# Michaelszeng/GCS-ADMM

Measured on NVIDIA B200. Metric: admm_iterations_per_second, higher is better.
Workload: dtype f64

## Files before the change

gcs-admm_b200/csrc/emulate.cpp:

```cpp
#define GCS_EMULATE 1
#include <stdio.h>
#include <stdlib.h>
#include <string.h>
#include "vertex_update.cuh"
#include "vertex_perf.cuh"

extern "C" int gcsemu_vertex_update_all(int nV, int nE, const int *poly_off, const double *polyA, const double *polyb,
                                        const int *he_off, const int *he_edge, const unsigned char *he_flags,
                                        const unsigned char *vtype, const double *cent, double *xc, const double *mu,
                                        const double *z, double *x_v, double *z_v, double *y_v, double rho, double mu_scale,
                                        double tol, int max_iter, int dcap, int mcap, long *total_iters, double *ws, double theta) {
    GcsGraphView G = {nV, nE, poly_off, polyA, polyb, he_off, he_edge, he_flags, vtype, cent};
    GcsStateView St = {xc, mu, z, x_v, z_v, y_v, ws, theta, 0.0};
    GcsScratchLayout L = gcs_scratch_layout(dcap, mcap);
    double *S = (double *)malloc(sizeof(double) * L.total);
    int fails = 0;
    long iters = 0;
    for (int v = 0; v < nV; ++v) {
        int status = 0;
        memset(S, getenv("GCSEMU_POISON") ? 0xFF : 0, sizeof(double) * L.total);
        iters += gcs_vertex_update(G, St, v, rho, mu_scale, tol, max_iter, L, S, 0, &status);
        if (status > 0 && status != 5) { fails++; if (getenv("GCSEMU_VERBOSE")) fprintf(stderr, "emu: vertex %d status %d\n", v, status); }
    }
    free(S);
    *total_iters = iters;
    return fails;
}
extern "C" int gcsemu_scratch_doubles(int dcap, int mcap) { return gcs_scratch_layout(dcap, mcap).total; }
extern "C" int gcsemu_ws_stride(int dcap, int mcap) { return gcs_ws_stride(gcs_scratch_layout(dcap, mcap)); }

template <bool INNER>
static int perf_all(int nV, int nE, const int *poly_off, const double *polyA, const double *polyb,
                    const int *he_off, const int *he_edge, const unsigned char *he_flags,
                    const unsigned char *vtype, const double *cent, double *xc, const double *mu,
                    const double *z, double *x_v, double *z_v, double *y_v, double rho, double mu_scale,
                    const int *vclass, const double *cls_tab, const int *cone_off, const double *cone,
                    const int *blk_off, const int *blk_he, const int *blk_edge, const int *blk_info, const int *tile_voff, int ntiles,
                    int cap_blocks, int cap_verts, int cap_cone, double *tstate, double *tn,
                    int inner_iters, double alpha, double kappa, double theta, const double *edge_delta, double *rin_tile) {
    GcsGraphView G = {nV, nE, poly_off, polyA, polyb, he_off, he_edge, he_flags, vtype, cent};
    GcsStateView St = {xc, mu, z, x_v, z_v, y_v, 0, 0.0, 0.0};
    GcsPerfLayout L = gcs_perf_layout(cap_blocks, cap_verts, cap_cone);
    const int nB = blk_off[nV];
    int *brec = (int *)calloc(4 * (size_t)(nB ? nB : 1), sizeof(int)), *vrec = (int *)calloc(GCS_VI_N * (size_t)nV, sizeof(int)), *trec = (int *)calloc(8 * (size_t)ntiles, sizeof(int));
    for (int b = 0; b < nB; ++b) { brec[4 * b] = blk_he[b]; brec[4 * b + 1] = blk_info[b]; brec[4 * b + 2] = blk_edge[b]; }
    for (int t = 0; t < ntiles; ++t) {
        const int a = tile_voff[t], b = tile_voff[t + 1];
        int *r = trec + 8 * t;
        r[0] = a; r[1] = b - a; r[2] = blk_off[a]; r[3] = blk_off[b] - blk_off[a]; r[4] = cone_off[a]; r[5] = cone_off[b] - cone_off[a];
        r[6] = he_off[a]; r[7] = he_off[b] - he_off[a];
        for (int hh = he_off[a]; hh < he_off[b]; ++hh) if (he_flags[hh] & GCS_HE_ZERO) r[7] |= 1 << 30;
        for (int v = a; v < b; ++v) {
            int *w = vrec + GCS_VI_N * v;
            w[GCS_VI_CONE] = cone_off[v] - cone_off[a]; w[GCS_VI_NV] = cone_off[v + 1] - cone_off[v]; w[GCS_VI_CLS] = vclass[v];
            w[GCS_VI_TERM] = vtype[v] != GCS_VT_GENERIC; w[GCS_VI_BLK] = blk_off[v] - blk_off[a]; w[GCS_VI_NB] = blk_off[v + 1] - blk_off[v];
            w[GCS_VI_ACTIVE] = 0; w[GCS_VI_HE] = he_off[v] - he_off[a];
        }
    }
    GcsPerfTables T = {vclass, cls_tab, cone_off, cone, blk_off, brec, vrec, trec, ntiles, tstate, tn, inner_iters, alpha, kappa, theta, edge_delta};
    Ctrl ctrl;
    memset(&ctrl, 0, sizeof ctrl);
    ctrl.rho = rho; ctrl.mu_scale = mu_scale;
    const int poison = getenv("GCSEMU_POISON") ? 0xFF : 0;
#pragma omp parallel
    {
        double *S = (double *)malloc(sizeof(double) * L.total);
#pragma omp for schedule(dynamic, 16)
        for (int t = 0; t < ntiles; ++t) {
            memset(S, poison, sizeof(double) * L.total);
            Ctrl local = ctrl;
            double rin = 0.0;
            gcs_perf_tile<INNER>(G, St, T, L, S, S + L.work, t, &local, 0, rin);
            if (rin_tile) rin_tile[t] = rin;
        }
        free(S);
    }
    free(brec); free(vrec); free(trec);
    for (int v = 0; v < nV; ++v)
        if (vtype[v] == GCS_VT_DEAD) { for (int k = 0; k < 4; ++k) { z_v[4 * v + k] = 0.0; x_v[4 * v + k] = cent[2 * v + (k & 1)]; } y_v[v] = 0.0; }
    return ntiles;
}

extern "C" int gcsemu_vertex_update_perf_all(int nV, int nE, const int *poly_off, const double *polyA, const double *polyb,
                                             const int *he_off, const int *he_edge, const unsigned char *he_flags,
                                             const unsigned char *vtype, const double *cent, double *xc, const double *mu,
                                             const double *z, double *x_v, double *z_v, double *y_v, double rho, double mu_scale,
                                             const int *vclass, const double *cls_tab, const int *cone_off, const double *cone,
                                             const int *blk_off, const int *blk_he, const int *blk_edge, const int *blk_info, const int *tile_voff, int ntiles,
                                             int cap_blocks, int cap_verts, int cap_cone, double *tstate, double *tn,
                                             int inner_iters, double alpha, double kappa, double theta, const double *edge_delta) {
    return perf_all<false>(nV, nE, poly_off, polyA, polyb, he_off, he_edge, he_flags, vtype, cent, xc, mu, z, x_v, z_v, y_v, rho, mu_scale,
                           vclass, cls_tab, cone_off, cone, blk_off, blk_he, blk_edge, blk_info, tile_voff, ntiles, cap_blocks, cap_verts,
                           cap_cone, tstate, tn, inner_iters, alpha, kappa, theta, edge_delta, nullptr);
}

extern "C" int gcsemu_vertex_update_perf_inner(int nV, int nE, const int *poly_off, const double *polyA, const double *polyb,
                                               const int *he_off, const int *he_edge, const unsigned char *he_flags,
                                               const unsigned char *vtype, const double *cent, double *xc, const double *mu,
                                               const double *z, double *x_v, double *z_v, double *y_v, double rho, double mu_scale,
                                               const int *vclass, const double *cls_tab, const int *cone_off, const double *cone,
                                               const int *blk_off, const int *blk_he, const int *blk_edge, const int *blk_info, const int *tile_voff, int ntiles,
                                               int cap_blocks, int cap_verts, int cap_cone, double *tstate, double *tn,
                                               int inner_iters, double alpha, double kappa, double theta, const double *edge_delta, double *inner_sq) {
    double *rin = (double *)calloc((size_t)(ntiles > 0 ? ntiles : 1), sizeof(double));
    const int r = perf_all<true>(nV, nE, poly_off, polyA, polyb, he_off, he_edge, he_flags, vtype, cent, xc, mu, z, x_v, z_v, y_v, rho, mu_scale,
                                 vclass, cls_tab, cone_off, cone, blk_off, blk_he, blk_edge, blk_info, tile_voff, ntiles, cap_blocks, cap_verts,
                                 cap_cone, tstate, tn, inner_iters, alpha, kappa, theta, edge_delta, rin);
    double s = 0.0;
    for (int t = 0; t < ntiles; ++t) s += rin[t];
    *inner_sq = s;
    free(rin);
    return r;
}

extern "C" void gcsemu_cone_project(const double *cone, int nv, const double *pts, int n, double *out) {
    for (int i = 0; i < n; ++i) gcs_cone_project(cone, nv, pts[3 * i], pts[3 * i + 1], pts[3 * i + 2], out[3 * i], out[3 * i + 1], out[3 * i + 2]);
}
```

gcs-admm_b200/csrc/gcsadmm.cu:

```cuda
#include <cuda_runtime.h>
#include <math.h>
#include <stdio.h>
#include <stdlib.h>
#include <string.h>
#include <new>
#include <nvtx3/nvToolsExt.h>

struct NvtxRange {
    explicit NvtxRange(const char *name) { nvtxRangePushA(name); }
    ~NvtxRange() { nvtxRangePop(); }
};

#include "../../include/gcsadmm.h"
#include "gcs_ctrl.h"
#include "vertex_update.cuh"
#include "vertex_perf.cuh"

#define GCS_VERSION "gcsadmm 0.1.0 (sm_100a)"
#define K1_MAX_WARPS 12
#define EDGE_THREADS 256

static thread_local char g_err[512] = "";
static int set_err(int code, const char *fmt, const char *a = "", const char *b = "") {
    snprintf(g_err, sizeof g_err, fmt, a, b);
    return code;
}
#define CK(call)                                                                                   \
    do {                                                                                           \
        cudaError_t e_ = (call);                                                                   \
        if (e_ != cudaSuccess) return set_err(GCS_E_CUDA, "%s: %s", #call, cudaGetErrorString(e_)); \
    } while (0)

#define GCS_MAX_PEERS 8
#define GCS_PEER_TIMEOUT_NS 20000000000ull
struct PeerComm {
    int halo_flag[GCS_MAX_PEERS];
    int sums_flag[GCS_MAX_PEERS];
    double sums_in[2][GCS_MAX_PEERS][NSUMS];
    int k;
    int error;
};
struct PeerView {
    int rank, world;
    unsigned neighbours;
    double *xc[GCS_MAX_PEERS];
    PeerComm *comm[GCS_MAX_PEERS];
    int nHown[GCS_MAX_PEERS], nHghost[GCS_MAX_PEERS];
};

struct PeerPush { const int *send_he, *send_rank, *send_slot; int nsend; const PeerView *PV; unsigned int *ticket; };

struct GcsHandle {
    int device;
    cudaStream_t stream, own_stream;
    GcsParams p;
    int nV, nE, nHown, nHghost;
    int nP;
    long long n_x, n_mu;
    int dcap, mcap;
    GcsScratchLayout L;
    int k1_smem, k1_blocks, k1_warps, edge_blocks, edge_per_edge, edge_minb, edge_coop, coop_blocks;
    int *poly_off, *he_off, *he_edge, *edge_he_tail, *edge_he_head;
    double *polyA, *polyb, *cent;
    unsigned char *he_flags, *vtype, *edge_counted;
    int *vprob, *prob_eoff; long long *prob_nx, *prob_nmu;
    int *he_prob_host;
    unsigned int *ticket;
    unsigned int *push_ticket;
    double *xc, *mu, *z, *x_v, *z_v, *y_v;
    double *ws;
    double *partials;
    double *hist;
    int hist_cap;
    Ctrl *ctrl;
    Ctrl *ctrl_host;
    cudaEvent_t ev[4];
    void *flush_buf; size_t flush_bytes;
    int perf_on, perf_smem, perf_threads, perf_grid;
    int inner_on;
    GcsPerfLayout PL;
    GcsPerfTables PT;
    long long perf_nblocks;
    int *p_vclass, *p_cone_off, *p_blk_off, *p_blk_rec, *p_vrec, *p_tile_rec; double *p_cls_tab, *p_cone, *p_tstate, *p_tn, *p_edge_delta, *p_edge_cent, *p_tile_res;
    cudaGraphExec_t graph_exec; int graph_iters;
    int peer_on, rank, world, nsend;
    PeerView PV; PeerView *PV_dev;
    PeerComm *comm;
    void *ipc_opened[2 * GCS_MAX_PEERS];
    int *send_he, *send_rank, *send_slot;
};

__global__ void __launch_bounds__(K1_MAX_WARPS * 32)
vertex_kernel(GcsGraphView G, GcsStateView St, Ctrl *ctrl_all, const int *__restrict__ vprob, GcsScratchLayout L, double tol, int max_iter) {
    extern __shared__ double smem[];
    const int lane = threadIdx.x & 31, warp = threadIdx.x >> 5;
    const int v = blockIdx.x * (blockDim.x >> 5) + warp;
    if (v >= G.nV) return;
    Ctrl *ctrl = ctrl_all + (vprob ? vprob[v] : 0);
    if (ctrl->stop && !ctrl->ignore_stop) return;
    double *S = smem + (size_t)warp * L.total;
    int status = 0;
    const int iters = gcs_vertex_update(G, St, v, ctrl->rho, ctrl->mu_scale, tol, max_iter, L, S, lane, &status);
    if (lane == 0) {
        if (iters) atomicAdd(&ctrl->inner_iters, (unsigned long long)iters);
        if (status > 0 && status != 5) atomicAdd(&ctrl->inner_fail, 1);
        if (status < 0) atomicAdd(&ctrl->skipped, 1ull);
    }
}

__device__ __forceinline__ unsigned long long gcs_globaltimer() { unsigned long long t; asm volatile("mov.u64 %0, %globaltimer;" : "=l"(t)); return t; }

__device__ __forceinline__ void peer_push(const double *xc, const int *__restrict__ send_he, const int *__restrict__ send_rank,
                                          const int *__restrict__ send_slot, int nsend, const PeerView &PV) {
    const int k = PV.comm[PV.rank]->k + 1, par = k & 1;
    for (int i = threadIdx.x; i < 5 * nsend; i += blockDim.x) {
        const int j = i / 5, c = i - 5 * j, q = send_rank[j];
        PV.xc[q][5 * ((size_t)PV.nHown[q] + (size_t)par * PV.nHghost[q] + send_slot[j]) + c] = __ldcg(xc + 5 * (size_t)send_he[j] + c);
    }
    __threadfence_system();
    __syncthreads();
    if (threadIdx.x < PV.world && ((PV.neighbours >> threadIdx.x) & 1u)) *(volatile int *)&PV.comm[threadIdx.x]->halo_flag[PV.rank] = k;
}
__device__ __forceinline__ void peer_wait_halo(const PeerView &PV) {
    PeerComm *me = PV.comm[PV.rank];
    const int k = me->k + 1, p = threadIdx.x;
    if (p < PV.world && ((PV.neighbours >> p) & 1u)) {
        const unsigned long long t0 = gcs_globaltimer();
        while (*(volatile int *)&me->halo_flag[p] < k)
            if (gcs_globaltimer() - t0 > GCS_PEER_TIMEOUT_NS) { me->error = 1; break; }
        __threadfence_system();
    }
    __syncthreads();
}

template <bool INNER>
__global__ void __launch_bounds__(GCS_PERF_THREADS, 4)
vertex_perf_kernel(GcsGraphView G, GcsStateView St, GcsPerfTables T, Ctrl *ctrl_all, const int *__restrict__ vprob, GcsPerfLayout L, PeerPush P) {
    extern __shared__ __align__(16) double smem[];
    __shared__ __align__(8) unsigned long long bar[2];
    if (!vprob && ctrl_all->stop && !ctrl_all->ignore_stop) return;
    int tile = blockIdx.x;
    if (tile >= T.ntiles) return;
    double *const stage0 = smem + L.work;
#define STAGE(b) (stage0 + (b) * L.stage)
    if (threadIdx.x == 0) {
        gcs_mbar_init(&bar[0], 1);
        gcs_mbar_init(&bar[1], 1);
        gcs_perf_stage(T, L, STAGE(0), tile, &bar[0]);
    }
    __syncthreads();
    unsigned phase = 0;
    double rin = 0.0;
    for (int buf = 0; tile < T.ntiles; tile += gridDim.x, buf ^= 1) {
        const int next = tile + gridDim.x;
        if (threadIdx.x == 0 && next < T.ntiles) {
            gcs_bulk_wait_read();
            gcs_perf_stage(T, L, STAGE(buf ^ 1), next, &bar[buf ^ 1]);
        }
        gcs_mbar_wait(&bar[buf], (phase >> buf) & 1u);
        phase ^= 1u << buf;
        gcs_perf_tile<INNER>(G, St, T, L, smem, STAGE(buf), tile, ctrl_all, vprob, rin);
    }
    if (threadIdx.x == 0) gcs_bulk_wait_read();
#undef STAGE
    if (INNER) {
#pragma unroll
        for (int o = 16; o; o >>= 1) rin += __shfl_xor_sync(0xffffffffu, rin, o);
        __syncthreads();
        if ((threadIdx.x & 31) == 0) smem[L.rin + (threadIdx.x >> 5)] = rin;
        __syncthreads();
        if (threadIdx.x == 0) {
            double s = 0.0;
            for (int w2 = 0; w2 < (int)(blockDim.x >> 5); ++w2) s += smem[L.rin + w2];
            T.tile_res[blockIdx.x] = s;
        }
    }
    if (P.PV) {
        __shared__ int is_last;
        __threadfence();
        __syncthreads();
        if (threadIdx.x == 0) is_last = (atomicAdd(P.ticket, 1u) == gridDim.x - 1);
        __syncthreads();
        if (is_last) {
            __threadfence();
            peer_push(St.xc, P.send_he, P.send_rank, P.send_slot, P.nsend, *P.PV);
            if (threadIdx.x == 0) *P.ticket = 0u;
        }
    }
}
__global__ void perf_init_dead_kernel(GcsGraphView G, GcsStateView St) {
    const int v = blockIdx.x * blockDim.x + threadIdx.x;
    if (v >= G.nV || G.vtype[v] != GCS_VT_DEAD) return;
    for (int k = 0; k < 4; ++k) { St.z_v[4 * (size_t)v + k] = 0.0; St.x_v[4 * (size_t)v + k] = G.cent[2 * (size_t)v + (k & 1)]; }
    St.y_v[v] = 0.0;
}

__device__ void control_apply(Ctrl *ctrl, const GcsParams &p, long long n_x, long long n_mu, double *hist, int hist_cap) {
    const int it = ctrl->it + 1;
    const double *s = ctrl->sums;
    const double rho = ctrl->rho;
    const double pri = sqrt(s[0]);
    const double dual = rho * sqrt(2.0 * s[1]);
    double rho_new = rho, scale = 1.0;
    const bool may = it < p.frac * p.max_it && (p.adapt_every <= 1 || it % p.adapt_every == 0);
    if (pri >= p.nu * dual && may) { rho_new = rho * p.tau_incr; scale = 1.0 / p.tau_incr; }
    else if (dual >= p.nu * pri && may) { rho_new = rho * (1.0 / p.tau_decr); scale = p.tau_incr; }
    const double nAx = sqrt(s[2]), nBz = sqrt(2.0 * s[3]), nmu = scale * sqrt(s[4]);
    const double eps_pri = sqrt((double)n_x) * p.eps_abs + p.eps_rel * fmax(nAx, nBz);
    const double eps_dual = sqrt((double)n_mu) * p.eps_abs + p.eps_rel * nmu;
    const double inner = s[6] < 0.0 ? -1.0 : sqrt(s[6]);
    const double pri_g = s[7] < 0.0 ? -1.0 : sqrt(s[7]), dual_g = s[8] < 0.0 ? -1.0 : rho * sqrt(2.0 * s[8]);
    ctrl->pri_g = pri_g; ctrl->dual_g = dual_g;
    ctrl->it = it; ctrl->pri = pri; ctrl->dual = dual; ctrl->eps_pri = eps_pri; ctrl->eps_dual = eps_dual; ctrl->inner = inner;
    ctrl->rho = rho_new; ctrl->mu_scale = scale;
    if (it < hist_cap) { hist[it] = rho_new; hist[hist_cap + it] = pri; hist[2 * hist_cap + it] = dual; }
    if (s[5] != 0.0 || !isfinite(pri) || !isfinite(dual)) { ctrl->diverged = 1; ctrl->stop = 1; return; }
    const bool ref = p.stop_ref && pri_g >= 0.0 && dual_g >= 0.0;
    const bool opt = p.abs_stop ? (inner >= 0.0 && fmax(fmax(ref ? pri_g : pri, ref ? dual_g : dual), inner) < p.abs_tol)
                                : (pri < eps_pri && dual < eps_dual);
    if (opt) { ctrl->opt = 1; ctrl->stop = 1; }
}

__device__ __forceinline__ void edge_finish(double r2, double dz2, double x2, double z2, double m2, double r2g, double dz2g, Ctrl *ctrl, double *__restrict__ partials,
                                            unsigned int *ticket, int fuse, const GcsParams &p, long long n_x, long long n_mu, double *hist,
                                            int hist_cap, const PeerView *PVp, const double *__restrict__ tile_res, int ntiles) {
    double bad = 0;
    if (!isfinite(r2) || !isfinite(dz2) || !isfinite(x2) || !isfinite(z2)) bad = 1.0;
    __shared__ double sh[EDGE_THREADS][9];
    __shared__ int is_last;
    double vals[8] = {r2, dz2, x2, z2, m2, bad, r2g, dz2g};
#pragma unroll
    for (int q = 0; q < 8; ++q)
#pragma unroll
        for (int o = 16; o; o >>= 1) vals[q] += __shfl_xor_sync(0xffffffffu, vals[q], o);
    const int lane = threadIdx.x & 31, warp = threadIdx.x >> 5;
    if (lane == 0)
#pragma unroll
        for (int q = 0; q < 8; ++q) sh[warp][q] = vals[q];
    __syncthreads();
    if (threadIdx.x < 8) {
        double s = 0.0;
        for (int w2 = 0; w2 < EDGE_THREADS / 32; ++w2) s += sh[w2][threadIdx.x];
        partials[(size_t)blockIdx.x * NSUMS + (threadIdx.x < 6 ? threadIdx.x : threadIdx.x + 1)] = s;
        __threadfence();
    }
    __syncthreads();
    if (threadIdx.x == 0) {
        const unsigned int t = atomicAdd(ticket, 1u);
        is_last = (t == gridDim.x - 1);
    }
    __syncthreads();
    if (!is_last) return;
    __threadfence();
    double acc[9] = {0, 0, 0, 0, 0, 0, 0, 0, 0};
    for (int b = threadIdx.x; b < (int)gridDim.x; b += blockDim.x)
#pragma unroll
        for (int q = 0; q < 9; ++q) if (q != 6) acc[q] += __ldcg(partials + (size_t)b * NSUMS + q);
    if (tile_res) { for (int b = threadIdx.x; b < ntiles; b += blockDim.x) acc[6] += __ldcg(tile_res + b); }
    else if (ntiles < 0 && threadIdx.x == 0) acc[6] = -1.0;
#pragma unroll
    for (int q = 0; q < 9; ++q) sh[threadIdx.x][q] = acc[q];
    __syncthreads();
    for (int st = EDGE_THREADS / 2; st > 0; st >>= 1) {
        if (threadIdx.x < st)
#pragma unroll
            for (int q = 0; q < 9; ++q) sh[threadIdx.x][q] += sh[threadIdx.x + st][q];
        __syncthreads();
    }
    if (threadIdx.x < 9) ctrl->sums[threadIdx.x] = sh[0][threadIdx.x];
    __syncthreads();
    if (fuse == 2) {
        const int me = PVp->rank, world = PVp->world, k = PVp->comm[me]->k + 1, par = k & 1;
        if (threadIdx.x < 9)
            for (int q = 0; q < world; ++q) PVp->comm[q]->sums_in[par][me][threadIdx.x] = sh[0][threadIdx.x];
        __threadfence_system();
        __syncthreads();
        if (threadIdx.x < world) { *(volatile int *)&PVp->comm[threadIdx.x]->sums_flag[me] = k; }
        if (threadIdx.x == 0) *ticket = 0u;
        return;
    }
    if (threadIdx.x == 0) {
        *ticket = 0u;
        if (fuse) control_apply(ctrl, p, n_x, n_mu, hist, hist_cap);
    }
}

__global__ void __launch_bounds__(EDGE_THREADS, 6)
edge_kernel(int nE, int nHown, const int *__restrict__ edge_he_tail, const int *__restrict__ edge_he_head,
            const unsigned char *__restrict__ edge_counted, const double *__restrict__ xc, double *__restrict__ mu,
            double *__restrict__ z, Ctrl *ctrl, double *__restrict__ partials, unsigned int *ticket, int fuse,
            GcsParams p, long long n_x, long long n_mu, double *hist, int hist_cap, int nHghost, const PeerView *PVp, const double *__restrict__ tile_res, int ntiles) {
    if (ctrl->stop && !ctrl->ignore_stop) return;
    if (fuse == 2) peer_wait_halo(*PVp);
    const double ms = ctrl->mu_scale, oa = p.outer_alpha, ob = 1.0 - p.outer_alpha;
    const int gpar = fuse == 2 ? ((PVp->comm[PVp->rank]->k + 1) & 1) * nHghost : 0;
    double r2 = 0, dz2 = 0, x2 = 0, z2 = 0, m2 = 0;
    const unsigned n = 5u * (unsigned)nE, stride = gridDim.x * blockDim.x;
    for (unsigned i = blockIdx.x * blockDim.x + threadIdx.x; i < n; i += stride) {
        const unsigned e = i / 5u, c = i - 5u * e;
        const int ht = edge_he_tail[e], hh = edge_he_head[e];
        const bool ot = ht < nHown, oh = hh < nHown;
        const unsigned it_ = 5u * (unsigned)(ot ? ht : ht + gpar) + c, ih_ = 5u * (unsigned)(oh ? hh : hh + gpar) + c;
        const double xt = xc[it_], xh = xc[ih_], zo = z[i];
        const double mt = ot ? mu[it_] : 0.0, mh = oh ? mu[ih_] : 0.0;
        const double w = edge_counted ? (double)edge_counted[e] : 1.0;
        double at = xt, ah = xh;
        if (oa != 1.0) { at = oa * xt + ob * zo; ah = oa * xh + ob * zo; }
        const double zn = 0.5 * (at + ah), dd = zn - zo;
        z[i] = zn;
        dz2 += w * dd * dd; z2 += w * zn * zn;
        if (ot) { const double r = zn - xt, mn = ms * mt + (zn - at); mu[it_] = mn; r2 += r * r; x2 += xt * xt; m2 += mn * mn; }
        if (oh) { const double r = zn - xh, mn = ms * mh + (zn - ah); mu[ih_] = mn; r2 += r * r; x2 += xh * xh; m2 += mn * mn; }
    }
    const double none = (blockIdx.x == 0 && threadIdx.x == 0) ? -1.0 : 0.0;
    edge_finish(r2, dz2, x2, z2, m2, none, none, ctrl, partials, ticket, fuse, p, n_x, n_mu, hist, hist_cap, PVp, tile_res, ntiles);
}

template <int MINB, bool OA, bool GRES>
__global__ void __launch_bounds__(EDGE_THREADS, MINB)
edge_frames_kernel(int nE, int nHown, const int *__restrict__ edge_he_tail, const int *__restrict__ edge_he_head,
                   const unsigned char *__restrict__ edge_counted, const double *__restrict__ edge_delta, const double *__restrict__ edge_cent, const double *__restrict__ xc,
                   double *__restrict__ mu, double *__restrict__ z, Ctrl *ctrl, double *__restrict__ partials, unsigned int *ticket, int fuse,
                   GcsParams p, long long n_x, long long n_mu, double *hist, int hist_cap, int nHghost, const PeerView *PVp, const double *__restrict__ tile_res, int ntiles) {
    if (ctrl->stop && !ctrl->ignore_stop) return;
    if (fuse == 2) peer_wait_halo(*PVp);
    const double ms = ctrl->mu_scale, oa = p.outer_alpha, ob = 1.0 - p.outer_alpha;
    const int gpar = fuse == 2 ? ((PVp->comm[PVp->rank]->k + 1) & 1) * nHghost : 0;
    double r2 = 0, dz2 = 0, x2 = 0, z2 = 0, m2 = 0, r2g = 0, dz2g = 0;
    if (!GRES && blockIdx.x == 0 && threadIdx.x == 0) r2g = dz2g = -1.0;
    const int estride = gridDim.x * blockDim.x;
    int e = blockIdx.x * blockDim.x + threadIdx.x, ht = 0, hh = 0;
    if (e < nE) { ht = edge_he_tail[e]; hh = edge_he_head[e]; }
    for (; e < nE; e += estride) {
        const int en = e + estride, ht_ = ht, hh_ = hh;
        if (en < nE) { ht = edge_he_tail[en]; hh = edge_he_head[en]; }
        const bool ot = ht_ < nHown, oh = hh_ < nHown;
        const double *pt = xc + 5 * (size_t)(ot ? ht_ : ht_ + gpar), *ph = xc + 5 * (size_t)(oh ? hh_ : hh_ + gpar);
        double xt[5], xh[5], zo[5], mt[5], mh[5];
#pragma unroll
        for (int c = 0; c < 5; ++c) { xt[c] = pt[c]; xh[c] = ph[c]; zo[c] = z[5 * (size_t)e + c]; }
        if (MINB == 2) {
#pragma unroll
            for (int c = 0; c < 5; ++c) { mt[c] = ot ? mu[5 * (size_t)ht_ + c] : 0.0; mh[c] = oh ? mu[5 * (size_t)hh_ + c] : 0.0; }
        }
        const double d0 = edge_delta ? edge_delta[2 * (size_t)e] : 0.0, d1 = edge_delta ? edge_delta[2 * (size_t)e + 1] : 0.0;
        const double w = edge_counted ? (double)edge_counted[e] : 1.0;
        double zn[5], bz[5], at[5], ah[5];
#pragma unroll
        for (int c = 0; c < 5; ++c) { at[c] = xt[c]; ah[c] = xh[c]; }
        if (OA) {
            const double bo[5] = {zo[0], zo[1], zo[2] - d0 * zo[4], zo[3] - d1 * zo[4], zo[4]};
#pragma unroll
            for (int c = 0; c < 5; ++c) { at[c] = oa * xt[c] + ob * bo[c]; ah[c] = oa * xh[c] + ob * zo[c]; }
        }
        zn[0] = 0.5 * (ah[0] + at[0]); zn[1] = 0.5 * (ah[1] + at[1]);
        const double q0 = ah[2] + at[2], q1 = ah[3] + at[3], q2 = ah[4] + at[4] - (d0 * at[2] + d1 * at[3]);
        zn[4] = (q2 + 0.5 * (d0 * q0 + d1 * q1)) / (2.0 + 0.5 * (d0 * d0 + d1 * d1));
        zn[2] = 0.5 * (q0 + d0 * zn[4]); zn[3] = 0.5 * (q1 + d1 * zn[4]);
        bz[0] = zn[0]; bz[1] = zn[1]; bz[2] = zn[2] - d0 * zn[4]; bz[3] = zn[3] - d1 * zn[4]; bz[4] = zn[4];
        double dd[5];
#pragma unroll
        for (int c = 0; c < 5; ++c) { dd[c] = zn[c] - zo[c]; z[5 * (size_t)e + c] = zn[c]; }
        const double db2 = dd[2] - d0 * dd[4], db3 = dd[3] - d1 * dd[4];
        dz2 += 0.5 * w * (2.0 * (dd[0] * dd[0] + dd[1] * dd[1] + dd[4] * dd[4]) + dd[2] * dd[2] + dd[3] * dd[3] + db2 * db2 + db3 * db3);
        z2 += 0.5 * w * (2.0 * (zn[0] * zn[0] + zn[1] * zn[1] + zn[4] * zn[4]) + zn[2] * zn[2] + zn[3] * zn[3] + bz[2] * bz[2] + bz[3] * bz[3]);
        double cu0 = 0.0, cu1 = 0.0, cw0 = 0.0, cw1 = 0.0;
        if (GRES) {
            cu0 = edge_cent[2 * (size_t)e]; cu1 = edge_cent[2 * (size_t)e + 1]; cw0 = cu0 - d0; cw1 = cu1 - d1;
            const double g0 = dd[0] + dd[4] * cu0, g1 = dd[1] + dd[4] * cu1, g2 = dd[2] + dd[4] * cw0, g3 = dd[3] + dd[4] * cw1;
            dz2g += w * (g0 * g0 + g1 * g1 + g2 * g2 + g3 * g3 + dd[4] * dd[4]);
        }
        if (MINB > 2) asm volatile("" ::: "memory");
        if (ot) {
            if (MINB > 2) {
#pragma unroll
                for (int c = 0; c < 5; ++c) mt[c] = mu[5 * (size_t)ht_ + c];
            }
#pragma unroll
            for (int c = 0; c < 5; ++c) { const double r = bz[c] - xt[c], mn = ms * mt[c] + (bz[c] - at[c]); mu[5 * (size_t)ht_ + c] = mn; r2 += r * r; x2 += xt[c] * xt[c]; m2 += mn * mn; }
            if (GRES) {
                const double ry = bz[4] - xt[4], a0 = bz[0] - xt[0] + ry * cu0, a1 = bz[1] - xt[1] + ry * cu1, a2 = bz[2] - xt[2] + ry * cu0, a3 = bz[3] - xt[3] + ry * cu1;
                r2g += a0 * a0 + a1 * a1 + a2 * a2 + a3 * a3 + ry * ry;
            }
        }
        if (oh) {
            if (MINB > 2) {
#pragma unroll
                for (int c = 0; c < 5; ++c) mh[c] = mu[5 * (size_t)hh_ + c];
            }
#pragma unroll
            for (int c = 0; c < 5; ++c) { const double r = zn[c] - xh[c], mn = ms * mh[c] + (zn[c] - ah[c]); mu[5 * (size_t)hh_ + c] = mn; r2 += r * r; x2 += xh[c] * xh[c]; m2 += mn * mn; }
            if (GRES) {
                const double ry = zn[4] - xh[4], a0 = zn[0] - xh[0] + ry * cu0, a1 = zn[1] - xh[1] + ry * cu1, a2 = zn[2] - xh[2] + ry * cw0, a3 = zn[3] - xh[3] + ry * cw1;
                r2g += a0 * a0 + a1 * a1 + a2 * a2 + a3 * a3 + ry * ry;
            }
        }
    }
    edge_finish(r2, dz2, x2, z2, m2, r2g, dz2g, ctrl, partials, ticket, fuse, p, n_x, n_mu, hist, hist_cap, PVp, tile_res, ntiles);
}

#define COOP_WARPS (EDGE_THREADS / 32)
#define COOP_SMEM_DOUBLES (COOP_WARPS * 5 * 160)
template <bool OA, int MINB>
__global__ void __launch_bounds__(EDGE_THREADS, MINB)
edge_coop_kernel(int nE, const int *__restrict__ edge_he_tail, const int *__restrict__ edge_he_head, const double *__restrict__ edge_delta,
                 const double *__restrict__ xc, double *__restrict__ mu, double *__restrict__ z, Ctrl *ctrl, double *__restrict__ partials,
                 unsigned int *ticket, int fuse, GcsParams p, long long n_x, long long n_mu, double *hist, int hist_cap,
                 const double *__restrict__ tile_res, int ntiles) {
    extern __shared__ __align__(16) double coop_sm[];
    if (ctrl->stop && !ctrl->ignore_stop) return;
    const double ms = ctrl->mu_scale, oa = p.outer_alpha, ob = 1.0 - p.outer_alpha;
    const int lane = threadIdx.x & 31, warp = threadIdx.x >> 5;
    double *xtS = coop_sm + (size_t)warp * 800, *xhS = xtS + 160, *zoS = xtS + 320, *mtS = xtS + 480, *mhS = xtS + 640;
    double r2 = 0, dz2 = 0, x2 = 0, z2 = 0, m2 = 0, r2g = 0, dz2g = 0;
    if (blockIdx.x == 0 && threadIdx.x == 0) r2g = dz2g = -1.0;
    const int nchunks = (nE + 31) >> 5;
    for (int chunk = blockIdx.x * COOP_WARPS + warp; chunk < nchunks; chunk += gridDim.x * COOP_WARPS) {
        const int e = (chunk << 5) + lane;
        const bool valid = e < nE;
        const int ht = valid ? edge_he_tail[e] : 0, hh = valid ? edge_he_head[e] : 0;
        const double d0 = valid && edge_delta ? edge_delta[2 * (size_t)e] : 0.0, d1 = valid && edge_delta ? edge_delta[2 * (size_t)e + 1] : 0.0;
        const size_t zbase = (size_t)chunk * 160;
        double vx[5], vh[5], vz[5], vm[5], vn[5];
        int tj[5], hj[5];
#pragma unroll
        for (int k = 0; k < 5; ++k) {
            const int i = lane + 32 * k, j = i / 5, c = i - 5 * j;
            tj[k] = 5 * __shfl_sync(0xffffffffu, ht, j) + c;
            hj[k] = 5 * __shfl_sync(0xffffffffu, hh, j) + c;
        }
#pragma unroll
        for (int k = 0; k < 5; ++k) {
            const int i = lane + 32 * k;
            vx[k] = xc[tj[k]]; vh[k] = xc[hj[k]]; vm[k] = mu[tj[k]]; vn[k] = mu[hj[k]];
            vz[k] = zbase + i < 5 * (size_t)nE ? z[zbase + i] : 0.0;
        }
#pragma unroll
        for (int k = 0; k < 5; ++k) {
            const int i = lane + 32 * k;
            xtS[i] = vx[k]; xhS[i] = vh[k]; mtS[i] = vm[k]; mhS[i] = vn[k]; zoS[i] = vz[k];
        }
        __syncwarp();
        double xt[5], xh[5], zo[5], mt[5], mh[5];
#pragma unroll
        for (int c = 0; c < 5; ++c) { xt[c] = xtS[5 * lane + c]; xh[c] = xhS[5 * lane + c]; zo[c] = zoS[5 * lane + c]; mt[c] = mtS[5 * lane + c]; mh[c] = mhS[5 * lane + c]; }
        __syncwarp();
        double zn[5], bz[5], at[5], ah[5];
#pragma unroll
        for (int c = 0; c < 5; ++c) { at[c] = xt[c]; ah[c] = xh[c]; }
        if (OA) {
            const double bo[5] = {zo[0], zo[1], zo[2] - d0 * zo[4], zo[3] - d1 * zo[4], zo[4]};
#pragma unroll
            for (int c = 0; c < 5; ++c) { at[c] = oa * xt[c] + ob * bo[c]; ah[c] = oa * xh[c] + ob * zo[c]; }
        }
        zn[0] = 0.5 * (ah[0] + at[0]); zn[1] = 0.5 * (ah[1] + at[1]);
        const double q0 = ah[2] + at[2], q1 = ah[3] + at[3], q2 = ah[4] + at[4] - (d0 * at[2] + d1 * at[3]);
        zn[4] = (q2 + 0.5 * (d0 * q0 + d1 * q1)) / (2.0 + 0.5 * (d0 * d0 + d1 * d1));
        zn[2] = 0.5 * (q0 + d0 * zn[4]); zn[3] = 0.5 * (q1 + d1 * zn[4]);
        bz[0] = zn[0]; bz[1] = zn[1]; bz[2] = zn[2] - d0 * zn[4]; bz[3] = zn[3] - d1 * zn[4]; bz[4] = zn[4];
        double dd[5];
#pragma unroll
        for (int c = 0; c < 5; ++c) { dd[c] = zn[c] - zo[c]; zoS[5 * lane + c] = zn[c]; }
        const double db2 = dd[2] - d0 * dd[4], db3 = dd[3] - d1 * dd[4];
        if (valid) {
            dz2 += 0.5 * (2.0 * (dd[0] * dd[0] + dd[1] * dd[1] + dd[4] * dd[4]) + dd[2] * dd[2] + dd[3] * dd[3] + db2 * db2 + db3 * db3);
            z2 += 0.5 * (2.0 * (zn[0] * zn[0] + zn[1] * zn[1] + zn[4] * zn[4]) + zn[2] * zn[2] + zn[3] * zn[3] + bz[2] * bz[2] + bz[3] * bz[3]);
        }
#pragma unroll
        for (int c = 0; c < 5; ++c) {
            const double r = bz[c] - xt[c], mn = ms * mt[c] + (bz[c] - at[c]);
            mtS[5 * lane + c] = mn;
            if (valid) { r2 += r * r; x2 += xt[c] * xt[c]; m2 += mn * mn; }
        }
#pragma unroll
        for (int c = 0; c < 5; ++c) {
            const double r = zn[c] - xh[c], mn = ms * mh[c] + (zn[c] - ah[c]);
            mhS[5 * lane + c] = mn;
            if (valid) { r2 += r * r; x2 += xh[c] * xh[c]; m2 += mn * mn; }
        }
        __syncwarp();
#pragma unroll
        for (int k = 0; k < 5; ++k) {
            const int i = lane + 32 * k, j = i / 5;
            if ((chunk << 5) + j < nE) { z[zbase + i] = zoS[i]; mu[tj[k]] = mtS[i]; mu[hj[k]] = mhS[i]; }
        }
        __syncwarp();
    }
    edge_finish(r2, dz2, x2, z2, m2, r2g, dz2g, ctrl, partials, ticket, fuse, p, n_x, n_mu, hist, hist_cap, nullptr, tile_res, ntiles);
}

__global__ void __launch_bounds__(1024)
peer_push_kernel(const double *__restrict__ xc, const int *__restrict__ send_he, const int *__restrict__ send_rank,
                 const int *__restrict__ send_slot, int nsend, Ctrl *ctrl, const PeerView *PVp) {
    if (ctrl->stop && !ctrl->ignore_stop) return;
    peer_push(xc, send_he, send_rank, send_slot, nsend, *PVp);
}
__global__ void peer_control_kernel(Ctrl *ctrl, GcsParams p, long long n_x, long long n_mu, double *hist, int hist_cap, const PeerView *PVp) {
    if (ctrl->stop && !ctrl->ignore_stop) return;
    const PeerView &PV = *PVp;
    PeerComm *me = PV.comm[PV.rank];
    const int k = me->k + 1, par = k & 1, q = threadIdx.x;
    if (q < PV.world) {
        const unsigned long long t0 = gcs_globaltimer();
        while (*(volatile int *)&me->sums_flag[q] < k)
            if (gcs_globaltimer() - t0 > GCS_PEER_TIMEOUT_NS) { me->error = 1; break; }
    }
    __threadfence_system();
    __syncwarp();
    if (threadIdx.x == 0) {
        for (int j = 0; j < 9; ++j) {
            double s = 0.0;
            for (int r = 0; r < PV.world; ++r) s += *(volatile double *)&me->sums_in[par][r][j];
            ctrl->sums[j] = s;
        }
        if (me->error) { ctrl->diverged = 1; ctrl->stop = 1; }
        else control_apply(ctrl, p, n_x, n_mu, hist, hist_cap);
        me->k = k;
    }
}

__global__ void control_kernel(Ctrl *ctrl, GcsParams p, long long n_x, long long n_mu, double *hist, int hist_cap) {
    if (threadIdx.x != 0 || blockIdx.x != 0) return;
    if (ctrl->stop && !ctrl->ignore_stop) return;
    control_apply(ctrl, p, n_x, n_mu, hist, hist_cap);
}

#define BATCH_THREADS 128
__global__ void __launch_bounds__(BATCH_THREADS)
batched_edge_kernel(int nP, const int *__restrict__ prob_eoff, int nHown, const int *__restrict__ edge_he_tail,
                    const int *__restrict__ edge_he_head, const double *__restrict__ xc, double *__restrict__ mu,
                    double *__restrict__ z, Ctrl *ctrl_all, GcsParams p, const long long *__restrict__ prob_nx,
                    const long long *__restrict__ prob_nmu, double *hist, int hist_cap) {
    __shared__ double sh[BATCH_THREADS / 32][6];
    for (int q = blockIdx.x; q < nP; q += gridDim.x) {
        Ctrl *ctrl = ctrl_all + q;
        if (ctrl->stop && !ctrl->ignore_stop) continue;
        const double ms = ctrl->mu_scale;
        double r2 = 0, dz2 = 0, x2 = 0, z2 = 0, m2 = 0, bad = 0;
        for (int e = prob_eoff[q] + threadIdx.x; e < prob_eoff[q + 1]; e += blockDim.x) {
            const int ht = edge_he_tail[e], hh = edge_he_head[e];
            double xt[5], xh[5], zn[5];
#pragma unroll
            for (int c = 0; c < 5; ++c) { xt[c] = xc[5 * (size_t)ht + c]; xh[c] = xc[5 * (size_t)hh + c]; }
#pragma unroll
            for (int c = 0; c < 5; ++c) {
                const double zo = z[5 * (size_t)e + c];
                zn[c] = 0.5 * (xt[c] + xh[c]);
                const double dd = zn[c] - zo;
                dz2 += dd * dd; z2 += zn[c] * zn[c];
                z[5 * (size_t)e + c] = zn[c];
            }
#pragma unroll
            for (int c = 0; c < 5; ++c) {
                const double rt = zn[c] - xt[c], mt = ms * mu[5 * (size_t)ht + c] + rt;
                mu[5 * (size_t)ht + c] = mt; r2 += rt * rt; x2 += xt[c] * xt[c]; m2 += mt * mt;
                const double rh = zn[c] - xh[c], mh = ms * mu[5 * (size_t)hh + c] + rh;
                mu[5 * (size_t)hh + c] = mh; r2 += rh * rh; x2 += xh[c] * xh[c]; m2 += mh * mh;
            }
        }
        if (!isfinite(r2) || !isfinite(dz2) || !isfinite(x2) || !isfinite(z2)) bad = 1.0;
        double vals[6] = {r2, dz2, x2, z2, m2, bad};
#pragma unroll
        for (int k = 0; k < 6; ++k)
#pragma unroll
            for (int o = 16; o; o >>= 1) vals[k] += __shfl_xor_sync(0xffffffffu, vals[k], o);
        const int lane = threadIdx.x & 31, warp = threadIdx.x >> 5;
        if (lane == 0)
            for (int k = 0; k < 6; ++k) sh[warp][k] = vals[k];
        __syncthreads();
        if (threadIdx.x == 0) {
            for (int k = 0; k < 6; ++k) {
                double sum = 0.0;
                for (int w2 = 0; w2 < BATCH_THREADS / 32; ++w2) sum += sh[w2][k];
                ctrl->sums[k] = sum;
            }
            control_apply(ctrl, p, prob_nx[q], prob_nmu[q], hist + (size_t)q * 3 * hist_cap, hist_cap);
        }
        __syncthreads();
    }
}
__global__ void set_ignore_kernel(Ctrl *ctrl, int nP, int v) {
    for (int q = blockIdx.x * blockDim.x + threadIdx.x; q < nP; q += gridDim.x * blockDim.x) ctrl[q].ignore_stop = v;
}

extern "C" const char *gcsadmm_version(void) { return GCS_VERSION; }
extern "C" const char *gcsadmm_last_error(void) { return g_err; }
extern "C" int gcsadmm_device_count(void) {
    int n = 0;
    if (cudaGetDeviceCount(&n) != cudaSuccess) { cudaGetLastError(); return 0; }
    return n;
}
extern "C" void gcsadmm_default_params(GcsParams *p) {
    p->rho0 = 1.0; p->tau_incr = 2.0; p->tau_decr = 2.0; p->nu = 10.0; p->frac = 0.1;
    p->eps_abs = 1e-4; p->eps_rel = 1e-3; p->max_it = 1000; p->inner_tol = 1e-8; p->inner_max_iter = 60;
    p->check_every = 8; p->abs_stop = 0; p->abs_tol = 1e-4; p->warm_theta = 1e-3; p->zero_tol = 1e-12;
    p->outer_alpha = 1.0; p->use_graph = 1; p->adapt_every = 1; p->stop_ref = 0;
}
extern "C" int gcsadmm_scratch_bytes(int max_live_degree, int max_rows) {
    return (int)(gcs_scratch_layout(max_live_degree, max_rows).total * sizeof(double));
}

template <typename T>
static int upload(T **dst, const T *src, size_t n) {
    if (n == 0) n = 1, src = nullptr;
    cudaError_t e = cudaMalloc((void **)dst, n * sizeof(T));
    if (e != cudaSuccess) { char nb[32]; snprintf(nb, sizeof nb, "%zu", n * sizeof(T)); return set_err(GCS_E_NOMEM, "cudaMalloc(%s bytes): %s", nb, cudaGetErrorString(e)); }
    if (src) { e = cudaMemcpy(*dst, src, n * sizeof(T), cudaMemcpyHostToDevice); if (e != cudaSuccess) return set_err(GCS_E_CUDA, "cudaMemcpy H2D: %s", cudaGetErrorString(e)); }
    else cudaMemset(*dst, 0, n * sizeof(T));
    return 0;
}

static int reset_ctrl(GcsHandle *h) {
    Ctrl c; memset(&c, 0, sizeof c);
    c.rho = h->p.rho0; c.mu_scale = 1.0;
    double first[3] = {h->p.rho0, 0.0, 0.0};
    for (int q = 0; q < h->nP; ++q) {
        h->ctrl_host[q] = c;
        for (int k = 0; k < 3; ++k)
            CK(cudaMemcpyAsync(h->hist + ((size_t)q * 3 + k) * h->hist_cap, &first[k], sizeof(double), cudaMemcpyHostToDevice, h->stream));
    }
    CK(cudaMemcpyAsync(h->ctrl, h->ctrl_host, sizeof(Ctrl) * h->nP, cudaMemcpyHostToDevice, h->stream));
    CK(cudaStreamSynchronize(h->stream));
    return 0;
}

static void free_perf(GcsHandle *h) {
    void *pp[] = {h->p_vclass, h->p_cone_off, h->p_blk_off, h->p_blk_rec, h->p_vrec, h->p_tile_rec, h->p_cls_tab, h->p_cone, h->p_tstate, h->p_tn, h->p_edge_delta, h->p_edge_cent, h->p_tile_res};
    for (void *q : pp) if (q) cudaFree(q);
    h->p_vclass = h->p_cone_off = h->p_blk_off = h->p_blk_rec = h->p_vrec = h->p_tile_rec = nullptr;
    h->p_cls_tab = h->p_cone = h->p_tstate = h->p_tn = h->p_edge_delta = h->p_edge_cent = h->p_tile_res = nullptr;
    h->perf_on = 0;
}
static void drop_graph(GcsHandle *h) {
    if (h->graph_exec) { cudaGraphExecDestroy(h->graph_exec); h->graph_exec = nullptr; }
    h->graph_iters = 0;
}

extern "C" int gcsadmm_destroy(GcsHandle *h) {
    if (!h) return 0;
    cudaSetDevice(h->device);
    void *ptrs[] = {h->poly_off, h->he_off, h->he_edge, h->edge_he_tail, h->edge_he_head, h->polyA, h->polyb, h->cent,
                    h->he_flags, h->vtype, h->edge_counted, h->xc, h->mu, h->z, h->x_v, h->z_v, h->y_v, h->ws, h->partials, h->hist, h->ctrl,
                    h->vprob, h->prob_eoff, h->prob_nx, h->prob_nmu};
    for (void *p : ptrs) if (p) cudaFree(p);
    if (h->ctrl_host) cudaFreeHost(h->ctrl_host);
    free(h->he_prob_host);
    if (h->flush_buf) cudaFree(h->flush_buf);
    if (h->graph_exec) cudaGraphExecDestroy(h->graph_exec);
    for (void *m : h->ipc_opened) if (m) cudaIpcCloseMemHandle(m);
    { void *pp[] = {h->comm, h->send_he, h->send_rank, h->send_slot, h->PV_dev}; for (void *q : pp) if (q) cudaFree(q); }
    if (h->ticket) cudaFree(h->ticket);
    if (h->push_ticket) cudaFree(h->push_ticket);
    free_perf(h);
    for (int i = 0; i < 4; ++i) if (h->ev[i]) cudaEventDestroy(h->ev[i]);
    if (h->own_stream) cudaStreamDestroy(h->own_stream);
    delete h;
    return 0;
}

static int validate_graph(const GcsGraph *g) {
    if (!g->poly_off || !g->polyA || !g->polyb || !g->he_off || !g->vtype || !g->cent) return set_err(GCS_E_INVALID, "null graph array%s", "");
    if (g->nH_own < 0 || g->nH_ghost < 0 || g->he_off[0] != 0 || g->he_off[g->nV] != g->nH_own) return set_err(GCS_E_INVALID, "he_off does not span nH_own%s", "");
    if (g->nH_own && (!g->he_edge || !g->he_flags)) return set_err(GCS_E_INVALID, "null half-edge array%s", "");
    if (g->nE && (!g->edge_he_tail || !g->edge_he_head)) return set_err(GCS_E_INVALID, "null edge array%s", "");
    if (g->poly_off[0] != 0) return set_err(GCS_E_INVALID, "poly_off[0] != 0%s", "");
    for (int v = 0; v < g->nV; ++v) {
        if (g->he_off[v + 1] < g->he_off[v] || g->poly_off[v + 1] < g->poly_off[v]) return set_err(GCS_E_INVALID, "offsets not monotone%s", "");
        if (g->vtype[v] > 3) return set_err(GCS_E_INVALID, "bad vertex type%s", "");
    }
    for (int hh = 0; hh < g->nH_own; ++hh) if (g->he_edge[hh] < 0 || g->he_edge[hh] >= g->nE) return set_err(GCS_E_INVALID, "he_edge out of range%s", "");
    const int nHall = g->nH_own + g->nH_ghost;
    for (int e = 0; e < g->nE; ++e)
        if (g->edge_he_tail[e] < 0 || g->edge_he_tail[e] >= nHall || g->edge_he_head[e] < 0 || g->edge_he_head[e] >= nHall)
            return set_err(GCS_E_INVALID, "edge_he_tail / edge_he_head out of range%s", "");
    return 0;
}

static int create_impl(GcsHandle *h, const GcsGraph *g) {
    int dcap = 1, mcap = 1;
    for (int v = 0; v < g->nV; ++v) {
        int d = 0;
        for (int hh = g->he_off[v]; hh < g->he_off[v + 1]; ++hh) if (!(g->he_flags[hh] & GCS_HE_FLAG_ZERO)) d++;
        if (d > dcap) dcap = d;
        int m = g->poly_off[v + 1] - g->poly_off[v];
        if (m > mcap) mcap = m;
        if (g->vtype[v] == GCS_VT_GENERIC && d < 2) return set_err(GCS_E_INVALID, "inconsistent presolve flags (generic vertex with < 2 live half-edges)%s", "");
    }
    h->dcap = dcap; h->mcap = mcap;
    h->L = gcs_scratch_layout(dcap, mcap);
    cudaDeviceProp prop;
    CK(cudaGetDeviceProperties(&prop, h->device));
    {
        const size_t per_warp = (size_t)h->L.total * sizeof(double);
        const size_t budget = prop.sharedMemPerBlockOptin;
        int w = (int)(budget / per_warp);
        if (w < 1) return set_err(GCS_E_INVALID, "vertex program too large for shared memory (max live degree / polytope rows too high)%s", "");
        if (w > K1_MAX_WARPS) w = K1_MAX_WARPS;
        h->k1_warps = w;
        h->k1_smem = (int)(w * per_warp);
    }
    CK(cudaFuncSetAttribute(vertex_kernel, cudaFuncAttributeMaxDynamicSharedMemorySize, h->k1_smem));
    CK(cudaFuncSetAttribute(vertex_kernel, cudaFuncAttributePreferredSharedMemoryCarveout, 100));
    h->k1_blocks = (g->nV + h->k1_warps - 1) / h->k1_warps;
    {
        const long long need = (5ll * g->nE + EDGE_THREADS - 1) / EDGE_THREADS;
        const char *bps = getenv("GCS_EDGE_BLOCKS_PER_SM"), *ek = getenv("GCS_EDGE_KERNEL");
        h->edge_per_edge = !(ek && !strcmp(ek, "per_scalar"));
        h->edge_coop = !(ek && (!strcmp(ek, "per_edge") || !strcmp(ek, "per_scalar")));
        h->coop_blocks = prop.multiProcessorCount * (bps && atoi(bps) > 0 ? atoi(bps) : 2);
        const char *mb = getenv("GCS_EDGE_MINB");
        h->edge_minb = mb && atoi(mb) >= 2 && atoi(mb) <= 4 ? atoi(mb) : 2;
        if (h->edge_coop) {
            const int smb = (int)(sizeof(double) * COOP_SMEM_DOUBLES);
            CK(cudaFuncSetAttribute(edge_coop_kernel<false, 2>, cudaFuncAttributeMaxDynamicSharedMemorySize, smb));
            CK(cudaFuncSetAttribute(edge_coop_kernel<true, 2>, cudaFuncAttributeMaxDynamicSharedMemorySize, smb));
            CK(cudaFuncSetAttribute(edge_coop_kernel<false, 3>, cudaFuncAttributeMaxDynamicSharedMemorySize, smb));
            CK(cudaFuncSetAttribute(edge_coop_kernel<true, 3>, cudaFuncAttributeMaxDynamicSharedMemorySize, smb));
        }
        const long long cap = (long long)prop.multiProcessorCount * (bps && atoi(bps) > 0 ? atoi(bps) : (h->edge_per_edge ? 4 : 6));
        h->edge_blocks = (int)(need < 1 ? 1 : (need > cap ? cap : need));
    }
    CK(cudaStreamCreateWithFlags(&h->own_stream, cudaStreamNonBlocking));
    h->stream = h->own_stream;
    const size_t M = (size_t)g->poly_off[g->nV], Hall = (size_t)g->nH_own + g->nH_ghost;
    int rc = 0;
#define UP(field, src, n) if (!rc) rc = upload(&h->field, src, (size_t)(n))
    UP(poly_off, g->poly_off, g->nV + 1); UP(polyA, g->polyA, 2 * M); UP(polyb, g->polyb, M);
    UP(he_off, g->he_off, g->nV + 1); UP(he_edge, g->he_edge, g->nH_own); UP(he_flags, g->he_flags, g->nH_own);
    UP(edge_he_tail, g->edge_he_tail, g->nE); UP(edge_he_head, g->edge_he_head, g->nE);
    UP(vtype, g->vtype, g->nV); UP(cent, g->cent, 2 * (size_t)g->nV);
    if (g->edge_counted) UP(edge_counted, g->edge_counted, g->nE);
    UP(xc, (const double *)nullptr, 5 * (Hall + (size_t)g->nH_ghost));
    UP(mu, (const double *)nullptr, 5 * (size_t)g->nH_own); UP(z, (const double *)nullptr, 5 * (size_t)g->nE);
    UP(x_v, (const double *)nullptr, 4 * (size_t)g->nV); UP(z_v, (const double *)nullptr, 4 * (size_t)g->nV); UP(y_v, (const double *)nullptr, g->nV);
    if (h->p.warm_theta > 0.0) UP(ws, (const double *)nullptr, (size_t)g->nV * gcs_ws_stride(h->L));
    UP(partials, (const double *)nullptr, (size_t)h->edge_blocks * NSUMS);
    UP(ticket, (const unsigned int *)nullptr, 1);
    UP(push_ticket, (const unsigned int *)nullptr, 1);
    h->hist_cap = h->p.max_it + 2;
    UP(hist, (const double *)nullptr, 3 * (size_t)h->hist_cap * h->nP);
#undef UP
    if (rc) return rc;
    CK(cudaMalloc((void **)&h->ctrl, sizeof(Ctrl) * h->nP));
    CK(cudaMallocHost((void **)&h->ctrl_host, sizeof(Ctrl) * h->nP));
    if (h->nP > 1) {
        int *vp = (int *)malloc(sizeof(int) * g->nV);
        long long *nx = (long long *)malloc(sizeof(long long) * h->nP), *nm = (long long *)malloc(sizeof(long long) * h->nP);
        h->he_prob_host = (int *)malloc(sizeof(int) * (size_t)(g->nH_own > 0 ? g->nH_own : 1));
        if (!vp || !nx || !nm || !h->he_prob_host) { free(vp); free(nx); free(nm); return set_err(GCS_E_NOMEM, "out of host memory%s", ""); }
        for (int q = 0; q < h->nP; ++q) {
            for (int v = g->prob_voff[q]; v < g->prob_voff[q + 1]; ++v) {
                vp[v] = q;
                for (int hh = g->he_off[v]; hh < g->he_off[v + 1]; ++hh) h->he_prob_host[hh] = q;
            }
            const long long nv = g->prob_voff[q + 1] - g->prob_voff[q], ne = g->prob_eoff[q + 1] - g->prob_eoff[q];
            nx[q] = 9 * nv + 18 * ne; nm[q] = 10 * ne;
        }
        rc = upload(&h->vprob, vp, (size_t)g->nV);
        if (!rc) rc = upload(&h->prob_eoff, g->prob_eoff, (size_t)h->nP + 1);
        if (!rc) rc = upload(&h->prob_nx, nx, (size_t)h->nP);
        if (!rc) rc = upload(&h->prob_nmu, nm, (size_t)h->nP);
        free(vp); free(nx); free(nm);
        if (rc) return rc;
    }
    for (int i = 0; i < 4; ++i) CK(cudaEventCreate(&h->ev[i]));
    return reset_ctrl(h);
}

extern "C" int gcsadmm_create(const GcsGraph *g, const GcsParams *p, int device, GcsHandle **out) {
    NvtxRange nvtx_("gcsadmm_create");
    if (!g || !out) return set_err(GCS_E_INVALID, "null argument%s", "");
    *out = nullptr;
    if (g->n != 2) return set_err(GCS_E_INVALID, "the CUDA path is specialised to n = 2 (2-D GCS)%s", "");
    if (g->nV <= 0 || g->nE < 0) return set_err(GCS_E_INVALID, "empty graph%s", "");
    int rc = validate_graph(g);
    if (rc) return rc;
    int ndev = 0;
    if (cudaGetDeviceCount(&ndev) != cudaSuccess || ndev == 0) { cudaGetLastError(); return set_err(GCS_E_CUDA, "no CUDA device: libgcsadmm has no CPU path%s", ""); }
    if (device < 0 || device >= ndev) return set_err(GCS_E_INVALID, "bad device index%s", "");
    const int nP = g->nP > 1 ? g->nP : 1;
    if (nP > 1 && (g->nH_ghost > 0 || !g->prob_voff || !g->prob_eoff)) return set_err(GCS_E_INVALID, "batched problems need prob_voff / prob_eoff and cannot be vertex-partitioned%s", "");
    CK(cudaSetDevice(device));
    GcsHandle *h = new (std::nothrow) GcsHandle();
    if (!h) return set_err(GCS_E_NOMEM, "out of host memory%s", "");
    memset(h, 0, sizeof *h);
    h->device = device;
    if (p) h->p = *p; else gcsadmm_default_params(&h->p);
    if (h->p.check_every < 1) h->p.check_every = 1;
    if (!(h->p.outer_alpha > 0.0 && h->p.outer_alpha < 2.0)) h->p.outer_alpha = 1.0;
    h->nV = g->nV; h->nE = g->nE; h->nHown = g->nH_own; h->nHghost = g->nH_ghost;
    h->nP = nP;
    h->n_x = g->n_x_global ? g->n_x_global : 9LL * g->nV + 18LL * g->nE;
    h->n_mu = g->n_mu_global ? g->n_mu_global : 10LL * g->nE;
    rc = create_impl(h, g);
    if (rc) { gcsadmm_destroy(h); return rc; }
    *out = h;
    return 0;
}

extern "C" int gcsadmm_set_stream(GcsHandle *h, void *s, int external) {
    if (!h) return set_err(GCS_E_INVALID, "null handle%s", "");
    CK(cudaSetDevice(h->device));
    CK(cudaStreamSynchronize(h->stream));
    h->stream = external ? (cudaStream_t)s : h->own_stream;
    drop_graph(h);
    return 0;
}

static GcsGraphView graph_view(const GcsHandle *h) {
    GcsGraphView G; G.nV = h->nV; G.nE = h->nE; G.poly_off = h->poly_off; G.polyA = h->polyA; G.polyb = h->polyb;
    G.he_off = h->he_off; G.he_edge = h->he_edge; G.he_flags = h->he_flags; G.vtype = h->vtype; G.cent = h->cent;
    return G;
}
static GcsStateView state_view(const GcsHandle *h) {
    GcsStateView S; S.xc = h->xc; S.mu = h->mu; S.z = h->z; S.x_v = h->x_v; S.z_v = h->z_v; S.y_v = h->y_v;
    S.ws = h->ws; S.theta = h->p.warm_theta; S.zero_tol = h->p.zero_tol;
    return S;
}
static int launch_k1(GcsHandle *h) {
    if (h->perf_on) {
        PeerPush P = {h->send_he, h->send_rank, h->send_slot, h->nsend, h->peer_on ? h->PV_dev : nullptr, h->push_ticket};
        if (h->inner_on) vertex_perf_kernel<true><<<h->perf_grid, h->perf_threads, h->perf_smem, h->stream>>>(graph_view(h), state_view(h), h->PT, h->ctrl, h->vprob, h->PL, P);
        else vertex_perf_kernel<false><<<h->perf_grid, h->perf_threads, h->perf_smem, h->stream>>>(graph_view(h), state_view(h), h->PT, h->ctrl, h->vprob, h->PL, P);
        return 0;
    }
    vertex_kernel<<<h->k1_blocks, h->k1_warps * 32, h->k1_smem, h->stream>>>(graph_view(h), state_view(h), h->ctrl, h->vprob, h->L, h->p.inner_tol, h->p.inner_max_iter);
    return 0;
}
#define INNER_ARGS(h) ((h)->perf_on && (h)->inner_on ? (h)->p_tile_res : nullptr), ((h)->perf_on && (h)->nP == 1 ? ((h)->inner_on ? (h)->perf_grid : -1) : 0)
static int launch_edge(GcsHandle *h, int fuse) {
    if (h->nP > 1) {
        const int blocks = h->nP < 148 * 16 ? h->nP : 148 * 16;
        batched_edge_kernel<<<blocks, BATCH_THREADS, 0, h->stream>>>(h->nP, h->prob_eoff, h->nHown, h->edge_he_tail, h->edge_he_head, h->xc, h->mu, h->z,
                                                                     h->ctrl, h->p, h->prob_nx, h->prob_nmu, h->hist, h->hist_cap);
        return 0;
    }
    if (h->edge_coop && h->nHghost == 0 && !h->edge_counted && !(h->perf_on && h->inner_on)) {
        const int nchunks = (h->nE + 31) / 32;
        int blocks = (nchunks + COOP_WARPS - 1) / COOP_WARPS;
        if (blocks > h->coop_blocks) blocks = h->coop_blocks;
        if (blocks < 1) blocks = 1;
        const size_t sm = sizeof(double) * COOP_SMEM_DOUBLES;
#define EDGE_COOP(OA, MINB) edge_coop_kernel<OA, MINB><<<blocks, EDGE_THREADS, sm, h->stream>>>(h->nE, h->edge_he_tail, h->edge_he_head, h->perf_on ? h->p_edge_delta : nullptr, \
            h->xc, h->mu, h->z, h->ctrl, h->partials, h->ticket, fuse, h->p, h->n_x, h->n_mu, h->hist, h->hist_cap, INNER_ARGS(h))
        if (h->p.outer_alpha != 1.0) { if (h->edge_minb >= 3) EDGE_COOP(true, 3); else EDGE_COOP(true, 2); }
        else { if (h->edge_minb >= 3) EDGE_COOP(false, 3); else EDGE_COOP(false, 2); }
#undef EDGE_COOP
        return 0;
    }
    if ((h->perf_on && h->p_edge_delta) || h->edge_per_edge) {
        int blocks = (h->nE + EDGE_THREADS - 1) / EDGE_THREADS;
        if (blocks > h->edge_blocks) blocks = h->edge_blocks;
        if (blocks < 1) blocks = 1;
        const bool gres = h->perf_on && h->inner_on && h->p_edge_delta && h->p_edge_cent;
#define EDGE_FRAMES(MINB) if (gres) { if (h->p.outer_alpha != 1.0) EDGE_FRAMES_(MINB, true, true); else EDGE_FRAMES_(MINB, false, true); } \
                          else { if (h->p.outer_alpha != 1.0) EDGE_FRAMES_(MINB, true, false); else EDGE_FRAMES_(MINB, false, false); }
#define EDGE_FRAMES_(MINB, OA, GRES) edge_frames_kernel<MINB, OA, GRES><<<blocks, EDGE_THREADS, 0, h->stream>>>(h->nE, h->nHown, h->edge_he_tail, h->edge_he_head, h->edge_counted, \
            h->perf_on ? h->p_edge_delta : nullptr, h->perf_on ? h->p_edge_cent : nullptr, h->xc, h->mu, h->z, h->ctrl, h->partials, h->ticket, fuse, h->p, h->n_x, h->n_mu, h->hist, h->hist_cap, h->nHghost, h->PV_dev, INNER_ARGS(h))
        if (h->edge_minb == 4) { EDGE_FRAMES(4); } else if (h->edge_minb == 3) { EDGE_FRAMES(3); } else { EDGE_FRAMES(2); }
#undef EDGE_FRAMES
#undef EDGE_FRAMES_
        return 0;
    }
    edge_kernel<<<h->edge_blocks, EDGE_THREADS, 0, h->stream>>>(h->nE, h->nHown, h->edge_he_tail, h->edge_he_head, h->edge_counted, h->xc, h->mu, h->z, h->ctrl,
                                                                h->partials, h->ticket, fuse, h->p, h->n_x, h->n_mu, h->hist, h->hist_cap, h->nHghost, h->PV_dev, INNER_ARGS(h));
    return 0;
}
static int launch_ctrl(GcsHandle *h) {
    if (h->nP > 1) return 0;
    control_kernel<<<1, 32, 0, h->stream>>>(h->ctrl, h->p, h->n_x, h->n_mu, h->hist, h->hist_cap);
    return 0;
}
static void launch_rest(GcsHandle *h) {
    if (!h->peer_on) { launch_edge(h, 1); return; }
    if (!h->perf_on) peer_push_kernel<<<1, 1024, 0, h->stream>>>(h->xc, h->send_he, h->send_rank, h->send_slot, h->nsend, h->ctrl, h->PV_dev);
    launch_edge(h, 2);
    peer_control_kernel<<<1, 32, 0, h->stream>>>(h->ctrl, h->p, h->n_x, h->n_mu, h->hist, h->hist_cap, h->PV_dev);
}
static void launch_iteration(GcsHandle *h) { launch_k1(h); launch_rest(h); }
static int launch_chunk(GcsHandle *h, int iters) {
    NvtxRange nvtx_("gcsadmm: chunk of ADMM iterations");
    if (!h->p.use_graph || h->stream != h->own_stream || iters < 2 || iters != h->p.check_every) { for (int i = 0; i < iters; ++i) launch_iteration(h); return 0; }
    if (!h->graph_exec || h->graph_iters != iters) {
        drop_graph(h);
        cudaGraph_t graph = nullptr;
        CK(cudaStreamBeginCapture(h->stream, cudaStreamCaptureModeThreadLocal));
        for (int i = 0; i < iters; ++i) launch_iteration(h);
        CK(cudaStreamEndCapture(h->stream, &graph));
        cudaError_t e = cudaGraphInstantiate(&h->graph_exec, graph, 0);
        cudaGraphDestroy(graph);
        if (e != cudaSuccess) { h->graph_exec = nullptr; return set_err(GCS_E_CUDA, "cudaGraphInstantiate: %s", cudaGetErrorString(e)); }
        h->graph_iters = iters;
    }
    CK(cudaGraphLaunch(h->graph_exec, h->stream));
    return 0;
}
static int set_ignore_stop(GcsHandle *h, int v) {
    if (h->nP > 1) { set_ignore_kernel<<<(h->nP + 255) / 256, 256, 0, h->stream>>>(h->ctrl, h->nP, v); return 0; }
    CK(cudaMemcpyAsync((char *)h->ctrl + offsetof(Ctrl, ignore_stop), &v, sizeof(int), cudaMemcpyHostToDevice, h->stream));
    return 0;
}
static int fetch_ctrl(GcsHandle *h) {
    CK(cudaMemcpyAsync(h->ctrl_host, h->ctrl, sizeof(Ctrl) * h->nP, cudaMemcpyDeviceToHost, h->stream));
    CK(cudaStreamSynchronize(h->stream));
    CK(cudaGetLastError());
    return 0;
}
static void fill_status_one(const Ctrl *c, GcsStatus *st) {
    st->iterations = c->it; st->converged = c->opt; st->diverged = c->diverged; st->inner_fail = c->inner_fail;
    st->inner_iters = (int64_t)c->inner_iters; st->skipped = (int64_t)c->skipped; st->rho = c->rho; st->pri_res = c->pri; st->dual_res = c->dual;
    st->eps_pri = c->eps_pri; st->eps_dual = c->eps_dual; st->inner_res = c->inner; st->pri_res_ref = c->pri_g >= 0.0 ? c->pri_g : c->pri; st->dual_res_ref = c->dual_g >= 0.0 ? c->dual_g : c->dual;
}
static void fill_status(const GcsHandle *h, GcsStatus *st) {
    fill_status_one(h->ctrl_host, st);
    for (int q = 1; q < h->nP; ++q) {
        GcsStatus t; fill_status_one(h->ctrl_host + q, &t);
        if (t.iterations > st->iterations) st->iterations = t.iterations;
        st->converged = st->converged && t.converged; st->diverged = st->diverged || t.diverged;
        st->inner_fail += t.inner_fail; st->inner_iters += t.inner_iters; st->skipped += t.skipped;
        if (t.pri_res > st->pri_res) { st->pri_res = t.pri_res; st->eps_pri = t.eps_pri; }
        if (t.dual_res > st->dual_res) { st->dual_res = t.dual_res; st->eps_dual = t.eps_dual; }
        if (t.inner_res > st->inner_res) st->inner_res = t.inner_res;
        if (t.pri_res_ref > st->pri_res_ref) st->pri_res_ref = t.pri_res_ref;
        if (t.dual_res_ref > st->dual_res_ref) st->dual_res_ref = t.dual_res_ref;
    }
}
static bool all_stopped(const GcsHandle *h) {
    for (int q = 0; q < h->nP; ++q) if (!h->ctrl_host[q].stop) return false;
    return true;
}
static bool any_diverged(const GcsHandle *h) {
    for (int q = 0; q < h->nP; ++q) if (h->ctrl_host[q].diverged) return true;
    return false;
}

extern "C" int gcsadmm_vertex_update(GcsHandle *h) { if (!h) return set_err(GCS_E_INVALID, "null handle%s", ""); CK(cudaSetDevice(h->device)); launch_k1(h); CK(cudaGetLastError()); return 0; }
extern "C" int gcsadmm_edge_update(GcsHandle *h) { if (!h) return set_err(GCS_E_INVALID, "null handle%s", ""); CK(cudaSetDevice(h->device)); launch_edge(h, 0); CK(cudaGetLastError()); return 0; }
extern "C" int gcsadmm_control(GcsHandle *h) { if (!h) return set_err(GCS_E_INVALID, "null handle%s", ""); CK(cudaSetDevice(h->device)); launch_ctrl(h); CK(cudaGetLastError()); return 0; }
extern "C" int gcsadmm_sums_device_ptr(GcsHandle *h, void **p) { if (!h || !p) return set_err(GCS_E_INVALID, "null argument%s", ""); *p = (char *)h->ctrl + offsetof(Ctrl, sums); return 0; }
extern "C" int gcsadmm_xc_device_ptr(GcsHandle *h, void **p) { if (!h || !p) return set_err(GCS_E_INVALID, "null argument%s", ""); *p = h->xc; return 0; }

extern "C" int gcsadmm_step(GcsHandle *h, int k) {
    if (!h) return set_err(GCS_E_INVALID, "null handle%s", "");
    CK(cudaSetDevice(h->device));
    int rc = set_ignore_stop(h, 1); if (rc) return rc;
    while (k > 0) {
        const int chunk = k < h->p.check_every ? k : h->p.check_every;
        rc = launch_chunk(h, chunk); if (rc) return rc;
        k -= chunk;
    }
    rc = set_ignore_stop(h, 0); if (rc) return rc;
    CK(cudaGetLastError());
    return fetch_ctrl(h);
}

extern "C" int gcsadmm_run(GcsHandle *h, int max_iters, GcsStatus *st) {
    NvtxRange nvtx_("gcsadmm_run");
    if (!h) return set_err(GCS_E_INVALID, "null handle%s", "");
    CK(cudaSetDevice(h->device));
    int rc = fetch_ctrl(h); if (rc) return rc;
    int done = 0;
    while (done < max_iters && !all_stopped(h)) {
        int chunk = h->p.check_every;
        if (chunk > max_iters - done) chunk = max_iters - done;
        rc = launch_chunk(h, chunk); if (rc) return rc;
        CK(cudaGetLastError());
        rc = fetch_ctrl(h); if (rc) return rc;
        done += chunk;
        if (h->perf_on && h->nP == 1 && h->p.abs_stop) {
            const int want = fmax(h->ctrl_host->pri, h->ctrl_host->dual) < 4.0 * h->p.abs_tol;
            if (want != h->inner_on) { h->inner_on = want; drop_graph(h); }
        }
    }
    if (st) fill_status(h, st);
    if (any_diverged(h)) return set_err(GCS_E_DIVERGED, "non-finite residuals (divergence)%s", "");
    return 0;
}

extern "C" int gcsadmm_get_status(GcsHandle *h, GcsStatus *st) {
    if (!h || !st) return set_err(GCS_E_INVALID, "null argument%s", "");
    CK(cudaSetDevice(h->device));
    int rc = fetch_ctrl(h); if (rc) return rc;
    fill_status(h, st);
    return 0;
}

extern "C" int gcsadmm_get_problem_status(GcsHandle *h, int problem, GcsStatus *st) {
    if (!h || !st || problem < 0 || problem >= h->nP) return set_err(GCS_E_INVALID, "bad argument%s", "");
    CK(cudaSetDevice(h->device));
    int rc = fetch_ctrl(h); if (rc) return rc;
    fill_status_one(h->ctrl_host + problem, st);
    return 0;
}
extern "C" int gcsadmm_get_problem_history(GcsHandle *h, int problem, double *rho, double *pri, double *dual, int cap) {
    if (!h || problem < 0 || problem >= h->nP) return set_err(GCS_E_INVALID, "bad argument%s", "");
    CK(cudaSetDevice(h->device));
    int rc = fetch_ctrl(h); if (rc) return rc;
    int n = h->ctrl_host[problem].it + 1;
    if (n > h->hist_cap) n = h->hist_cap;
    if (n > cap) n = cap;
    double *dst[3] = {rho, pri, dual};
    for (int k = 0; k < 3; ++k) if (dst[k]) CK(cudaMemcpy(dst[k], h->hist + ((size_t)problem * 3 + k) * h->hist_cap, sizeof(double) * n, cudaMemcpyDeviceToHost));
    return n;
}
extern "C" int gcsadmm_get_history(GcsHandle *h, double *rho, double *pri, double *dual, int cap) {
    if (!h) return set_err(GCS_E_INVALID, "null handle%s", "");
    CK(cudaSetDevice(h->device));
    int rc = fetch_ctrl(h); if (rc) return rc;
    int n = h->ctrl_host->it + 1;
    if (n > h->hist_cap) n = h->hist_cap;
    if (n > cap) n = cap;
    double *dst[3] = {rho, pri, dual};
    for (int q = 0; q < 3; ++q) if (dst[q]) CK(cudaMemcpy(dst[q], h->hist + (size_t)q * h->hist_cap, sizeof(double) * n, cudaMemcpyDeviceToHost));
    return n;
}

extern "C" int gcsadmm_get_solution(GcsHandle *h, double *x_v, double *z_v, double *y_v, double *z_e) {
    NvtxRange nvtx_("gcsadmm_get_solution");
    if (!h) return set_err(GCS_E_INVALID, "null handle%s", "");
    CK(cudaSetDevice(h->device));
    CK(cudaStreamSynchronize(h->stream));
    if (x_v) CK(cudaMemcpy(x_v, h->x_v, sizeof(double) * 4 * h->nV, cudaMemcpyDeviceToHost));
    if (z_v) CK(cudaMemcpy(z_v, h->z_v, sizeof(double) * 4 * h->nV, cudaMemcpyDeviceToHost));
    if (y_v) CK(cudaMemcpy(y_v, h->y_v, sizeof(double) * h->nV, cudaMemcpyDeviceToHost));
    if (z_e) CK(cudaMemcpy(z_e, h->z, sizeof(double) * 5 * h->nE, cudaMemcpyDeviceToHost));
    return 0;
}

extern "C" int gcsadmm_get_state(GcsHandle *h, double *xc, double *mu, double *z, double *rho, int *it) {
    if (!h) return set_err(GCS_E_INVALID, "null handle%s", "");
    CK(cudaSetDevice(h->device));
    int rc = fetch_ctrl(h); if (rc) return rc;
    if (xc) CK(cudaMemcpy(xc, h->xc, sizeof(double) * 5 * ((size_t)h->nHown + h->nHghost), cudaMemcpyDeviceToHost));
    if (mu) {
        CK(cudaMemcpy(mu, h->mu, sizeof(double) * 5 * (size_t)h->nHown, cudaMemcpyDeviceToHost));
        if (h->nP > 1) { for (size_t hh = 0; hh < (size_t)h->nHown; ++hh) { const double s = h->ctrl_host[h->he_prob_host[hh]].mu_scale; if (s != 1.0) for (int c = 0; c < 5; ++c) mu[5 * hh + c] *= s; } }
        else { const double s = h->ctrl_host->mu_scale; if (s != 1.0) for (size_t i = 0; i < 5 * (size_t)h->nHown; ++i) mu[i] *= s; }
    }
    if (z) CK(cudaMemcpy(z, h->z, sizeof(double) * 5 * (size_t)h->nE, cudaMemcpyDeviceToHost));
    if (rho) *rho = h->ctrl_host->rho;
    if (it) *it = h->ctrl_host->it;
    return 0;
}

extern "C" int gcsadmm_set_state(GcsHandle *h, const double *xc, const double *mu, const double *z, double rho, int it) {
    if (!h) return set_err(GCS_E_INVALID, "null handle%s", "");
    CK(cudaSetDevice(h->device));
    int rc = fetch_ctrl(h); if (rc) return rc;
    if (xc) CK(cudaMemcpy(h->xc, xc, sizeof(double) * 5 * ((size_t)h->nHown + h->nHghost), cudaMemcpyHostToDevice));
    if (mu) CK(cudaMemcpy(h->mu, mu, sizeof(double) * 5 * (size_t)h->nHown, cudaMemcpyHostToDevice));
    if (z) CK(cudaMemcpy(h->z, z, sizeof(double) * 5 * (size_t)h->nE, cudaMemcpyHostToDevice));
    for (int q = 0; q < h->nP; ++q) { Ctrl &c = h->ctrl_host[q]; c.rho = rho; c.it = it; c.mu_scale = 1.0; c.stop = 0; c.opt = 0; c.diverged = 0; }
    CK(cudaMemcpy(h->ctrl, h->ctrl_host, sizeof(Ctrl) * h->nP, cudaMemcpyHostToDevice));
    return 0;
}

extern "C" int gcsadmm_time_steps(GcsHandle *h, int k, float *ms_total, float *ms_k1, float *ms_edge) {
    if (!h || !ms_total) return set_err(GCS_E_INVALID, "null argument%s", "");
    CK(cudaSetDevice(h->device));
    int rc = set_ignore_stop(h, 1); if (rc) return rc;
    CK(cudaStreamSynchronize(h->stream));
    float k1 = 0.f, ed = 0.f;
    const bool split = ms_k1 || ms_edge;
    CK(cudaEventRecord(h->ev[0], h->stream));
    for (int i = 0; i < k; ++i) {
        if (split) CK(cudaEventRecord(h->ev[1], h->stream));
        if (h->peer_on) launch_iteration(h); else launch_k1(h);
        if (split) CK(cudaEventRecord(h->ev[2], h->stream));
        if (!h->peer_on) launch_edge(h, 1);
        if (split) {
            CK(cudaEventRecord(h->ev[3], h->stream));
            CK(cudaEventSynchronize(h->ev[3]));
            float a = 0.f, b = 0.f;
            CK(cudaEventElapsedTime(&a, h->ev[1], h->ev[2])); CK(cudaEventElapsedTime(&b, h->ev[2], h->ev[3]));
            k1 += a; ed += b;
        }
    }
    CK(cudaEventRecord(h->ev[3], h->stream));
    CK(cudaEventSynchronize(h->ev[3]));
    CK(cudaEventElapsedTime(ms_total, h->ev[0], h->ev[3]));
    if (ms_k1) *ms_k1 = k1;
    if (ms_edge) *ms_edge = ed;
    rc = set_ignore_stop(h, 0); if (rc) return rc;
    CK(cudaGetLastError());
    return fetch_ctrl(h);
}

extern "C" int gcsadmm_time_window(GcsHandle *h, int k, long long flush_bytes, float *ms_iter, float *ms_k1) {
    NvtxRange nvtx_("gcsadmm_time_window");
    if (!h || !ms_iter || k < 1) return set_err(GCS_E_INVALID, "bad argument%s", "");
    CK(cudaSetDevice(h->device));
    if (flush_bytes > 0 && (!h->flush_buf || h->flush_bytes < (size_t)flush_bytes)) {
        if (h->flush_buf) cudaFree(h->flush_buf);
        h->flush_buf = nullptr;
        CK(cudaMalloc(&h->flush_buf, (size_t)flush_bytes));
        h->flush_bytes = (size_t)flush_bytes;
    }
    int rc = set_ignore_stop(h, 1); if (rc) return rc;
    cudaEvent_t *ev = (cudaEvent_t *)calloc(3 * (size_t)k, sizeof(cudaEvent_t));
    if (!ev) return set_err(GCS_E_NOMEM, "out of host memory%s", "");
    cudaError_t e = cudaSuccess;
    for (int i = 0; i < 3 * k && e == cudaSuccess; ++i) e = cudaEventCreate(&ev[i]);
    for (int i = 0; i < k && e == cudaSuccess; ++i) {
        if (flush_bytes > 0) cudaMemsetAsync(h->flush_buf, 0, (size_t)flush_bytes, h->stream);
        cudaEventRecord(ev[3 * i], h->stream);
        launch_k1(h);
        if (ms_k1) cudaEventRecord(ev[3 * i + 1], h->stream);
        launch_rest(h);
        e = cudaEventRecord(ev[3 * i + 2], h->stream);
    }
    if (e == cudaSuccess) e = cudaStreamSynchronize(h->stream);
    for (int i = 0; i < k && e == cudaSuccess; ++i) {
        e = cudaEventElapsedTime(&ms_iter[i], ev[3 * i], ev[3 * i + 2]);
        if (ms_k1 && e == cudaSuccess) e = cudaEventElapsedTime(&ms_k1[i], ev[3 * i], ev[3 * i + 1]);
    }
    for (int i = 0; i < 3 * k; ++i) if (ev[i]) cudaEventDestroy(ev[i]);
    free(ev);
    if (e != cudaSuccess) return set_err(GCS_E_CUDA, "time_window: %s", cudaGetErrorString(e));
    rc = set_ignore_stop(h, 0); if (rc) return rc;
    CK(cudaGetLastError());
    return fetch_ctrl(h);
}

extern "C" int gcsadmm_solve_host(const GcsGraph *g, const GcsParams *p, int device, int max_iters, GcsStatus *st,
                                  double *x_v, double *z_v, double *y_v, double *z_e,
                                  double *rho_seq, double *pri_seq, double *dual_seq, int hist_cap) {
    GcsHandle *h = nullptr;
    int rc = gcsadmm_create(g, p, device, &h);
    if (rc) return rc;
    GcsStatus local;
    rc = gcsadmm_run(h, max_iters, st ? st : &local);
    if (rc == 0 || rc == GCS_E_DIVERGED) {
        int rc2 = gcsadmm_get_solution(h, x_v, z_v, y_v, z_e);
        if (rc2 == 0 && (rho_seq || pri_seq || dual_seq)) { int n = gcsadmm_get_history(h, rho_seq, pri_seq, dual_seq, hist_cap); if (n < 0) rc2 = n; }
        if (rc == 0) rc = rc2;
    }
    gcsadmm_destroy(h);
    return rc;
}

extern "C" int gcsadmm_peer_export(GcsHandle *h, void *handles128) {
    if (!h || !handles128) return set_err(GCS_E_INVALID, "null argument%s", "");
    CK(cudaSetDevice(h->device));
    if (!h->comm) {
        CK(cudaMalloc((void **)&h->comm, sizeof(PeerComm)));
        CK(cudaMemset(h->comm, 0, sizeof(PeerComm)));
    }
    cudaIpcMemHandle_t a, b;
    CK(cudaIpcGetMemHandle(&a, h->xc));
    CK(cudaIpcGetMemHandle(&b, h->comm));
    memcpy(handles128, &a, 64); memcpy((char *)handles128 + 64, &b, 64);
    return 0;
}
extern "C" int gcsadmm_peer_connect(GcsHandle *h, int rank, int world, const void *all_handles, const int *peer_nHown, const int *peer_nHghost,
                                    int nsend, const int *send_he, const int *send_rank, const int *send_slot) {
    if (!h || !all_handles || !peer_nHown || !peer_nHghost || (nsend && (!send_he || !send_rank || !send_slot))) return set_err(GCS_E_INVALID, "null argument%s", "");
    if (world < 1 || world > GCS_MAX_PEERS || rank < 0 || rank >= world) return set_err(GCS_E_INVALID, "peer mode supports 1..8 ranks%s", "");
    if (h->nP > 1) return set_err(GCS_E_INVALID, "batched problems are not vertex-partitioned%s", "");
    if (!h->comm) return set_err(GCS_E_INVALID, "call gcsadmm_peer_export first%s", "");
    if (peer_nHown[rank] != h->nHown || peer_nHghost[rank] != h->nHghost) return set_err(GCS_E_INVALID, "peer table disagrees with this rank's sizes%s", "");
    CK(cudaSetDevice(h->device));
    CK(cudaStreamSynchronize(h->stream));
    drop_graph(h);
    PeerView V;
    memset(&V, 0, sizeof V);
    V.rank = rank; V.world = world;
    for (int j = 0; j < nsend; ++j) {
        const int q = send_rank[j];
        if (q < 0 || q >= world || q == rank || send_he[j] < 0 || send_he[j] >= h->nHown || send_slot[j] < 0 || send_slot[j] >= peer_nHghost[q])
            return set_err(GCS_E_INVALID, "bad halo send table%s", "");
        V.neighbours |= 1u << q;
    }
    for (int q = 0; q < world; ++q) {
        V.nHown[q] = peer_nHown[q]; V.nHghost[q] = peer_nHghost[q];
        if (q == rank) { V.xc[q] = h->xc; V.comm[q] = h->comm; continue; }
        cudaIpcMemHandle_t a, b;
        memcpy(&a, (const char *)all_handles + 128 * q, 64); memcpy(&b, (const char *)all_handles + 128 * q + 64, 64);
        void *px = nullptr, *pc = nullptr;
        CK(cudaIpcOpenMemHandle(&px, a, cudaIpcMemLazyEnablePeerAccess));
        h->ipc_opened[2 * q] = px;
        CK(cudaIpcOpenMemHandle(&pc, b, cudaIpcMemLazyEnablePeerAccess));
        h->ipc_opened[2 * q + 1] = pc;
        V.xc[q] = (double *)px; V.comm[q] = (PeerComm *)pc;
    }
    int rc = 0;
    if (!rc) rc = upload(&h->send_he, send_he, (size_t)nsend);
    if (!rc) rc = upload(&h->send_rank, send_rank, (size_t)nsend);
    if (!rc) rc = upload(&h->send_slot, send_slot, (size_t)nsend);
    if (rc) return rc;
    if (!h->PV_dev) CK(cudaMalloc((void **)&h->PV_dev, sizeof(PeerView)));
    CK(cudaMemcpy(h->PV_dev, &V, sizeof(PeerView), cudaMemcpyHostToDevice));
    h->nsend = nsend; h->rank = rank; h->world = world; h->PV = V; h->peer_on = 1;
    return 0;
}
extern "C" int gcsadmm_peer_error(GcsHandle *h) {
    if (!h || !h->comm) return 0;
    int e = 0;
    cudaSetDevice(h->device);
    cudaMemcpy(&e, (char *)h->comm + offsetof(PeerComm, error), sizeof(int), cudaMemcpyDeviceToHost);
    return e;
}

extern "C" int gcsadmm_flush_l2(GcsHandle *h, long long bytes) {
    if (!h) return set_err(GCS_E_INVALID, "null handle%s", "");
    CK(cudaSetDevice(h->device));
    if (bytes <= 0) bytes = 256ll << 20;
    if (!h->flush_buf || h->flush_bytes < (size_t)bytes) {
        if (h->flush_buf) cudaFree(h->flush_buf);
        h->flush_buf = nullptr;
        CK(cudaMalloc(&h->flush_buf, (size_t)bytes));
        h->flush_bytes = (size_t)bytes;
    }
    CK(cudaMemsetAsync(h->flush_buf, 0, (size_t)bytes, h->stream));
    return 0;
}

extern "C" int gcsadmm_enable_perf(GcsHandle *h, const GcsPerfConfig *c) {
    NvtxRange nvtx_("gcsadmm_enable_perf");
    if (!h || !c) return set_err(GCS_E_INVALID, "null argument%s", "");
    if (c->inner_iters < 1 || c->n_classes < 1 || c->n_tiles < 1 || c->n_blocks < 0 || !c->vclass || !c->cls_tab || !c->cone_off || !c->cone ||
        !c->blk_off || !c->tile_voff || (c->n_blocks && (!c->blk_he || !c->blk_info)))
        return set_err(GCS_E_INVALID, "incomplete perf-mode tables%s", "");
    if (!(c->alpha > 0.0 && c->alpha < 2.0) || !(c->kappa > 0.0)) return set_err(GCS_E_INVALID, "perf mode needs 0 < alpha < 2 and kappa > 0%s", "");
    if (c->tile_voff[0] != 0 || c->tile_voff[c->n_tiles] != h->nV || c->blk_off[0] != 0 || c->blk_off[h->nV] != c->n_blocks || c->cone_off[0] != 0)
        return set_err(GCS_E_INVALID, "perf-mode offsets do not span the graph%s", "");
    for (int t = 0; t < c->n_tiles; ++t) {
        const int a = c->tile_voff[t], b = c->tile_voff[t + 1];
        if (b <= a || b > h->nV || b - a > 255 || b - a > c->cap_verts || c->blk_off[b] - c->blk_off[a] > c->cap_blocks ||
            c->cone_off[b] - c->cone_off[a] > c->cap_cone || c->blk_off[b] < c->blk_off[a] || c->cone_off[b] < c->cone_off[a])
            return set_err(GCS_E_INVALID, "perf-mode tile exceeds the declared capacities%s", "");
    }
    for (int v = 0; v < h->nV; ++v) if (c->vclass[v] >= c->n_classes) return set_err(GCS_E_INVALID, "vclass out of range%s", "");
    for (int b = 0; b < c->n_blocks; ++b) if (c->blk_he[b] >= h->nHown) return set_err(GCS_E_INVALID, "blk_he out of range%s", "");
    CK(cudaSetDevice(h->device));
    CK(cudaStreamSynchronize(h->stream));
    drop_graph(h);
    free_perf(h);
    int rc = 0;
    const size_t ncone = (size_t)c->cone_off[h->nV];
    if (!rc) rc = upload(&h->p_vclass, c->vclass, (size_t)h->nV);
    if (!rc) rc = upload(&h->p_cls_tab, c->cls_tab, (size_t)c->n_classes * GCS_CLS_STRIDE);
    if (!rc) rc = upload(&h->p_cone_off, c->cone_off, (size_t)h->nV + 1);
    if (!rc) rc = upload(&h->p_cone, c->cone, GCS_CONE_REC * ncone);
    if (!rc) rc = upload(&h->p_blk_off, c->blk_off, (size_t)h->nV + 1);
    if (!rc) {
        const size_t nB = (size_t)c->n_blocks, nVt = (size_t)h->nV, nT = (size_t)c->n_tiles;
        int *brec = (int *)calloc(4 * (nB ? nB : 1), sizeof(int)), *vrec = (int *)calloc(GCS_VI_N * nVt, sizeof(int)), *trec = (int *)calloc(8 * nT, sizeof(int));
        int *he_edge = (int *)malloc(sizeof(int) * (size_t)(h->nHown > 0 ? h->nHown : 1)), *he_off = (int *)malloc(sizeof(int) * (nVt + 1));
        unsigned char *vtype = (unsigned char *)malloc(nVt), *he_flags = (unsigned char *)malloc((size_t)(h->nHown > 0 ? h->nHown : 1));
        int *vprob = (int *)calloc(nVt, sizeof(int));
        if (!brec || !vrec || !trec || !he_edge || !he_off || !vtype || !he_flags || !vprob) rc = set_err(GCS_E_NOMEM, "out of host memory%s", "");
        if (!rc) {
            cudaMemcpy(he_edge, h->he_edge, sizeof(int) * (size_t)h->nHown, cudaMemcpyDeviceToHost);
            cudaMemcpy(he_off, h->he_off, sizeof(int) * (nVt + 1), cudaMemcpyDeviceToHost);
            cudaMemcpy(vtype, h->vtype, nVt, cudaMemcpyDeviceToHost);
            cudaMemcpy(he_flags, h->he_flags, (size_t)h->nHown, cudaMemcpyDeviceToHost);
            if (h->vprob) cudaMemcpy(vprob, h->vprob, sizeof(int) * nVt, cudaMemcpyDeviceToHost);
            for (size_t b = 0; b < nB; ++b) {
                brec[4 * b] = c->blk_he[b]; brec[4 * b + 1] = c->blk_info[b]; brec[4 * b + 2] = c->blk_he[b] >= 0 ? he_edge[c->blk_he[b]] : -1;
            }
            for (int t = 0; t < c->n_tiles; ++t) {
                const int a = c->tile_voff[t], b = c->tile_voff[t + 1];
                int *r = trec + 8 * (size_t)t;
                r[0] = a; r[1] = b - a; r[2] = c->blk_off[a]; r[3] = c->blk_off[b] - c->blk_off[a];
                r[4] = c->cone_off[a]; r[5] = c->cone_off[b] - c->cone_off[a]; r[6] = he_off[a]; r[7] = he_off[b] - he_off[a];
                bool zero = false;
                for (int hh = he_off[a]; hh < he_off[b]; ++hh) zero = zero || (he_flags[hh] & GCS_HE_FLAG_ZERO);
                if (zero) r[7] |= 1 << 30;
                for (int v = a; v < b; ++v) {
                    int *w = vrec + GCS_VI_N * (size_t)v;
                    w[GCS_VI_CONE] = c->cone_off[v] - c->cone_off[a]; w[GCS_VI_NV] = c->cone_off[v + 1] - c->cone_off[v];
                    w[GCS_VI_CLS] = c->vclass[v]; w[GCS_VI_TERM] = vtype[v] != GCS_VT_GENERIC;
                    w[GCS_VI_BLK] = c->blk_off[v] - c->blk_off[a]; w[GCS_VI_NB] = c->blk_off[v + 1] - c->blk_off[v];
                    w[GCS_VI_ACTIVE] = vprob[v]; w[GCS_VI_HE] = he_off[v] - he_off[a];
                }
            }
            rc = upload(&h->p_blk_rec, brec, 4 * nB);
            if (!rc) rc = upload(&h->p_vrec, vrec, GCS_VI_N * nVt);
            if (!rc) rc = upload(&h->p_tile_rec, trec, 8 * nT);
        }
        free(brec); free(vrec); free(trec); free(he_edge); free(he_off); free(vtype); free(he_flags); free(vprob);
    }
    if (!rc) rc = upload(&h->p_tstate, (const double *)nullptr, 12 * (size_t)c->n_blocks);
    if (!rc) rc = upload(&h->p_tn, (const double *)nullptr, 2 * (size_t)h->nV);
    if (!rc) rc = upload(&h->p_tile_res, (const double *)nullptr, (size_t)c->n_tiles);
    if (!rc && c->edge_delta) rc = upload(&h->p_edge_delta, c->edge_delta, 2 * (size_t)h->nE);
    if (!rc && c->edge_delta && c->edge_cent) rc = upload(&h->p_edge_cent, c->edge_cent, 2 * (size_t)h->nE);
    if (rc) { free_perf(h); return rc; }
    h->perf_nblocks = c->n_blocks;
    h->PL = gcs_perf_layout(c->cap_blocks, c->cap_verts, c->cap_cone);
    h->PT.vclass = h->p_vclass; h->PT.cls_tab = h->p_cls_tab; h->PT.cone_off = h->p_cone_off; h->PT.cone = h->p_cone;
    h->PT.blk_off = h->p_blk_off; h->PT.blk_rec = h->p_blk_rec; h->PT.vrec = h->p_vrec; h->PT.tile_rec = h->p_tile_rec;
    h->PT.ntiles = c->n_tiles; h->PT.tstate = h->p_tstate; h->PT.tn = h->p_tn; h->PT.inner_iters = c->inner_iters;
    h->PT.alpha = c->alpha; h->PT.kappa = c->kappa; h->PT.theta = c->theta > 0.0 ? c->theta : 1.0; h->PT.edge_delta = h->p_edge_delta; h->PT.tile_res = h->p_tile_res;
    cudaDeviceProp prop;
    CK(cudaGetDeviceProperties(&prop, h->device));
    const size_t bytes = (size_t)(h->PL.work + 2 * h->PL.stage) * sizeof(double);
    if (bytes > prop.sharedMemPerBlockOptin) { free_perf(h); return set_err(GCS_E_INVALID, "perf-mode tile too large for shared memory (a vertex of very high degree)%s", ""); }
    h->perf_smem = (int)bytes;
    h->perf_threads = c->threads >= 32 && c->threads <= GCS_PERF_THREADS ? (c->threads / 32) * 32 : GCS_PERF_THREADS;
    {
        const char *bps = getenv("GCS_PERF_BLOCKS_PER_SM");
        int per_sm = bps && atoi(bps) > 0 ? atoi(bps) : 4;
        const int by_smem = (int)(prop.sharedMemPerMultiprocessor / (bytes + 1024));
        if (per_sm > by_smem) per_sm = by_smem > 0 ? by_smem : 1;
        const long long cap = (long long)prop.multiProcessorCount * per_sm;
        h->perf_grid = (int)(c->n_tiles < cap ? c->n_tiles : cap);
    }
    CK(cudaFuncSetAttribute(vertex_perf_kernel<false>, cudaFuncAttributeMaxDynamicSharedMemorySize, h->perf_smem));
    CK(cudaFuncSetAttribute(vertex_perf_kernel<false>, cudaFuncAttributePreferredSharedMemoryCarveout, 100));
    CK(cudaFuncSetAttribute(vertex_perf_kernel<true>, cudaFuncAttributeMaxDynamicSharedMemorySize, h->perf_smem));
    CK(cudaFuncSetAttribute(vertex_perf_kernel<true>, cudaFuncAttributePreferredSharedMemoryCarveout, 100));
    perf_init_dead_kernel<<<(h->nV + 255) / 256, 256, 0, h->stream>>>(graph_view(h), state_view(h));
    CK(cudaGetLastError());
    CK(cudaStreamSynchronize(h->stream));
    h->perf_on = 1;
    return 0;
}

extern "C" int gcsadmm_get_perf_state(GcsHandle *h, double *tstate, double *tn) {
    if (!h || !h->perf_on) return set_err(GCS_E_INVALID, "perf mode is not enabled%s", "");
    CK(cudaSetDevice(h->device));
    CK(cudaStreamSynchronize(h->stream));
    if (tstate && h->perf_nblocks) CK(cudaMemcpy(tstate, h->p_tstate, sizeof(double) * 12 * (size_t)h->perf_nblocks, cudaMemcpyDeviceToHost));
    if (tn) CK(cudaMemcpy(tn, h->p_tn, sizeof(double) * 2 * (size_t)h->nV, cudaMemcpyDeviceToHost));
    return 0;
}
extern "C" int gcsadmm_set_perf_state(GcsHandle *h, const double *tstate, const double *tn) {
    if (!h || !h->perf_on) return set_err(GCS_E_INVALID, "perf mode is not enabled%s", "");
    CK(cudaSetDevice(h->device));
    CK(cudaStreamSynchronize(h->stream));
    if (tstate && h->perf_nblocks) CK(cudaMemcpy(h->p_tstate, tstate, sizeof(double) * 12 * (size_t)h->perf_nblocks, cudaMemcpyHostToDevice));
    if (tn) CK(cudaMemcpy(h->p_tn, tn, sizeof(double) * 2 * (size_t)h->nV, cudaMemcpyHostToDevice));
    return 0;
}
```

gcs-admm_b200/csrc/vertex_perf.cuh:

```cuda
#pragma once
#include <string.h>
#include "gcs_ctrl.h"
#include "vertex_update.cuh"

#define GCS_CONE_REC 12
#define GCS_NCX 19
#define GCS_CLS_G0 361
#define GCS_CLS_DINV 380
#define GCS_CLS_STRIDE 392
#define GCS_PERF_THREADS 256

#ifdef GCS_EMULATE
#define GCS_CTA_LOOP(i, n) for (int i = 0; i < (n); ++i)
#define GCS_CTA_SYNC() ((void)0)
#else
#define GCS_CTA_LOOP(i, n) for (int i = threadIdx.x; i < (n); i += blockDim.x)
#define GCS_CTA_SYNC() __syncthreads()
#endif

struct GcsPerfTables {
    const int *vclass;
    const double *cls_tab;
    const int *cone_off;
    const double *cone;
    const int *blk_off;
    const int *blk_rec;
    const int *vrec;
    const int *tile_rec;
    int ntiles;
    double *tstate;
    double *tn;
    int inner_iters;
    double alpha, kappa;
    double theta;
    const double *edge_delta;
    double *tile_res;
};

struct GcsPerfLayout { int nb_cap, nvt_cap, cone_cap, tS, cone, tnS, vi, bi, tr, stage, eS, enS, T, r, cin, cout, vd, rin, work, total; };
#define GCS_VI_N 8
#define GCS_VI_CONE 0
#define GCS_VI_NV 1
#define GCS_VI_CLS 2
#define GCS_VI_TERM 3
#define GCS_VI_BLK 4
#define GCS_VI_NB 5
#define GCS_VI_ACTIVE 6
#define GCS_VI_HE 7
#if defined(__CUDACC__)
__host__ __device__
#endif
static inline GcsPerfLayout gcs_perf_layout(int nb_cap, int nvt_cap, int cone_cap) {
    GcsPerfLayout L;
    if (nb_cap < 1) nb_cap = 1;
    if (nvt_cap < 1) nvt_cap = 1;
    if (cone_cap < 1) cone_cap = 1;
    L.nb_cap = nb_cap; L.nvt_cap = nvt_cap; L.cone_cap = cone_cap;
    int o = 0;
    L.tS = o; o += 12 * nb_cap;
    L.cone = o; o += GCS_CONE_REC * cone_cap;
    L.tnS = o; o += 2 * nvt_cap;
    L.vi = o; o += (GCS_VI_N * nvt_cap) / 2;
    L.bi = o; o += 2 * nb_cap;
    L.tr = o; o += 4;
    L.stage = o;
    o = 0;
    L.eS = o; o += 12 * nb_cap;
    L.enS = o; o += 2 * nvt_cap;
    L.T = o; o += 5 * nb_cap;
    L.r = o; o += 5 * nb_cap;
    L.cin = o; o += GCS_NCX * nvt_cap;
    L.cout = o; o += GCS_NCX * nvt_cap;
    L.vd = o; o += 2 * nvt_cap;
    L.rin = o; o += GCS_PERF_THREADS / 32;
    L.work = o + (o & 1);
    L.total = L.work + L.stage;
    return L;
}

GCS_DEV void gcs_cone_project(const double *cone, int nv, double c0, double c1, double c2, double &q0, double &q1, double &q2) {
    double best = 0.0;
    int code = -1;
    bool inside = true;
    for (int k = 0; k < nv; ++k) {
#if defined(GCS_EMULATE)
        const double *r = cone + GCS_CONE_REC * k;
        const double vx = r[0], vy = r[1], nx = r[2], ny = r[3], nh = r[4], inv = r[5], a0 = r[6], a1 = r[7], a2 = r[8], b0 = r[9], b1 = r[10], b2 = r[11];
#else
        const double2 *r = reinterpret_cast<const double2 *>(cone + GCS_CONE_REC * k);
        const double2 r0 = r[0], r1 = r[1], r2 = r[2], r3 = r[3], r4 = r[4], r5 = r[5];
        const double vx = r0.x, vy = r0.y, nx = r1.x, ny = r1.y, nh = r2.x, inv = r2.y, a0 = r3.x, a1 = r3.y, a2 = r4.x, b0 = r4.y, b1 = r5.x, b2 = r5.y;
#endif
        const double tau = c0 * vx + c1 * vy + c2;
        const double dist = nx * c0 + ny * c1 + nh * c2;
        if (tau > 0.0) {
            const double red = tau * tau * inv;
            if (red > best) { best = red; code = 2 * k; }
        }
        if (dist > 0.0) {
            inside = false;
            if (c0 * a0 + c1 * a1 + c2 * a2 >= 0.0 && c0 * b0 + c1 * b1 + c2 * b2 >= 0.0) { best = 1e300; code = 2 * k + 1; }
        }
    }
    if (inside) { q0 = c0; q1 = c1; q2 = c2; return; }
    q0 = 0.0; q1 = 0.0; q2 = 0.0;
    if (code < 0) return;
    const double *ck = cone + GCS_CONE_REC * (code >> 1);
    if (code & 1) {
        const double dist = ck[2] * c0 + ck[3] * c1 + ck[4] * c2;
        q0 = c0 - dist * ck[2]; q1 = c1 - dist * ck[3]; q2 = c2 - dist * ck[4];
    } else {
        const double tau = (c0 * ck[0] + c1 * ck[1] + c2) * ck[5];
        q0 = tau * ck[0]; q1 = tau * ck[1]; q2 = tau;
    }
}

#if !defined(GCS_EMULATE) && defined(__CUDACC__)
__device__ __forceinline__ unsigned gcs_smem_u32(const void *p) { return (unsigned)__cvta_generic_to_shared(p); }
__device__ __forceinline__ void gcs_mbar_init(unsigned long long *bar, unsigned count) {
    asm volatile("mbarrier.init.shared::cta.b64 [%0], %1;" ::"r"(gcs_smem_u32(bar)), "r"(count) : "memory");
    asm volatile("fence.mbarrier_init.release.cluster;" ::: "memory");
}
__device__ __forceinline__ void gcs_mbar_expect_tx(unsigned long long *bar, unsigned bytes) {
    asm volatile("mbarrier.arrive.expect_tx.shared::cta.b64 _, [%0], %1;" ::"r"(gcs_smem_u32(bar)), "r"(bytes) : "memory");
}
__device__ __forceinline__ void gcs_bulk_g2s(void *dst, const void *src, unsigned bytes, unsigned long long *bar) {
    asm volatile("cp.async.bulk.shared::cluster.global.mbarrier::complete_tx::bytes [%0], [%1], %2, [%3];"
                 ::"r"(gcs_smem_u32(dst)), "l"(src), "r"(bytes), "r"(gcs_smem_u32(bar)) : "memory");
}
__device__ __forceinline__ void gcs_mbar_wait(unsigned long long *bar, unsigned parity) {
    unsigned done = 0;
    while (!done) {
        asm volatile("{\n .reg .pred p;\n mbarrier.try_wait.parity.shared::cta.b64 p, [%1], %2;\n selp.u32 %0, 1, 0, p;\n}"
                     : "=r"(done) : "r"(gcs_smem_u32(bar)), "r"(parity) : "memory");
    }
}
__device__ __forceinline__ void gcs_bulk_s2g(void *dst, const void *src, unsigned bytes) {
    asm volatile("cp.async.bulk.global.shared::cta.bulk_group [%0], [%1], %2;" ::"l"(dst), "r"(gcs_smem_u32(src)), "r"(bytes) : "memory");
}
__device__ __forceinline__ void gcs_bulk_commit() { asm volatile("cp.async.bulk.commit_group;" ::: "memory"); }
__device__ __forceinline__ void gcs_bulk_wait_read() { asm volatile("cp.async.bulk.wait_group.read 0;" ::: "memory"); }
__device__ __forceinline__ void gcs_fence_async_smem() { asm volatile("fence.proxy.async.shared::cta;" ::: "memory"); }
#endif

#define GCS_PF 3

GCS_DEV double gcs_core_input(const double *tS, const double *rS, const int *brec, const int *w, int k, double kappa) {
    const int bl = w[GCS_VI_BLK], zb = bl + w[GCS_VI_NB] - 1;
    double s = 0.0;
    if (k < 4) {
        if (!w[GCS_VI_TERM]) { for (int b = bl; b <= zb; ++b) s += tS[12 * b + 6 * (k >> 1) + 3 + (k & 1)]; s *= kappa; }
    } else if (k < 9) s = rS[5 * zb + k - 4];
    else {
        const int g = k >= 14, tau = k - 9 - 5 * g;
        for (int b = bl; b < zb; ++b) if (((brec[4 * b + 1] >> 8) & 3) == g) s += rS[5 * b + tau];
    }
    return s;
}
GCS_DEV double gcs_core_output(const double *tab, const double *in, int k) {
    const double *gk = tab + k;
    double s0 = tab[GCS_CLS_G0 + k], s1 = 0.0;
#pragma unroll
    for (int j = 0; j + 1 < GCS_NCX; j += 2) { s0 += gk[GCS_NCX * j] * in[j]; s1 += gk[GCS_NCX * (j + 1)] * in[j + 1]; }
    return s0 + s1 + gk[GCS_NCX * (GCS_NCX - 1)] * in[GCS_NCX - 1];
}

GCS_DEV double gcs_rhs(const GcsPerfTables &T, const double *tS, const double *TS, const double *tnS, const int *brec, int q, int vl, double rho, double kappa) {
    const int b = q / 5, tau = q - 5 * b, info = brec[4 * b + 1], grp = (info >> 8) & 3;
    const bool term = (info >> 10) & 1;
    const double *d = tS + 12 * b;
    double val;
    if (tau < 4) {
        const int i = tau >> 1, c = tau & 1;
        val = d[6 * i + c];
        if (!term) val -= d[6 * i + 3 + c];
        val *= kappa;
        if (grp == 1) val += TS[q];
        else if (grp == 0) { if (tau < 2) val += TS[q + 2]; }
        else val += (i ? -kappa : kappa) * tnS[2 * vl + c];
    } else {
        val = d[2] + d[8];
        if (!term) val += (1.0 - d[5]) + (1.0 - d[11]);
        val *= kappa;
        if (grp < 2) val += T.theta * TS[q] - GCS_EDGE_PENALTY / rho;
    }
    return val;
}
GCS_DEV double gcs_block_u(const double *rS, const double *co, const double *tab, int info, int b, int tau) {
    const int grp = (info >> 8) & 3;
    return grp == 2 ? co[4 + tau] : tab[GCS_CLS_DINV + 5 * grp + tau] * rS[5 * b + tau] + co[9 + 5 * grp + tau];
}

GCS_DEV double gcs_target_z(const GcsStateView &St, const GcsPerfTables &T, int e, int c, int info) {
    double zc = St.z[5 * (size_t)e + c];
    if (T.edge_delta && ((info >> 8) & 3) == 1 && (c == 2 || c == 3))
        zc -= T.edge_delta[2 * (size_t)e + c - 2] * St.z[5 * (size_t)e + 4];
    return zc;
}

#if !defined(GCS_EMULATE) && defined(__CUDACC__)
__device__ __forceinline__ void gcs_perf_stage(const GcsPerfTables &T, const GcsPerfLayout &L, double *B, int tile, unsigned long long *bar) {
    const int *tr = T.tile_rec + 8 * (size_t)tile;
    const int v0 = tr[0], nvt = tr[1], b0 = tr[2], nb = tr[3], c0 = tr[4], ncone = tr[5];
    gcs_mbar_expect_tx(bar, (unsigned)(sizeof(double) * (12 * nb + 2 * nvt + GCS_CONE_REC * ncone) + sizeof(int) * (GCS_VI_N * nvt + 4 * nb + 8)));
    gcs_bulk_g2s(B + L.tr, tr, (unsigned)(sizeof(int) * 8), bar);
    gcs_bulk_g2s(B + L.vi, T.vrec + GCS_VI_N * (size_t)v0, (unsigned)(sizeof(int) * GCS_VI_N * nvt), bar);
    if (nb) gcs_bulk_g2s(B + L.bi, T.blk_rec + 4 * (size_t)b0, (unsigned)(sizeof(int) * 4 * nb), bar);
    if (nb) gcs_bulk_g2s(B + L.tS, T.tstate + 12 * (size_t)b0, (unsigned)(sizeof(double) * 12 * nb), bar);
    gcs_bulk_g2s(B + L.tnS, T.tn + 2 * (size_t)v0, (unsigned)(sizeof(double) * 2 * nvt), bar);
    if (ncone) gcs_bulk_g2s(B + L.cone, T.cone + GCS_CONE_REC * (size_t)c0, (unsigned)(sizeof(double) * GCS_CONE_REC * ncone), bar);
}
#endif

template <bool INNER>
GCS_DEV void gcs_perf_tile(const GcsGraphView &G, const GcsStateView &St, const GcsPerfTables &T, const GcsPerfLayout &L,
                           double *S, double *B, int tile, Ctrl *ctrl_all, const int *vprob, double &rin) {
    const double rho_u = ctrl_all->rho, ms_u = ctrl_all->mu_scale;
#define RHO(vl) (vprob ? vd[2 * (vl)] : rho_u)
#define MSC(vl) (vprob ? vd[2 * (vl) + 1] : ms_u)
#define ACT(vl) (!vprob || vi[GCS_VI_N * (vl) + GCS_VI_ACTIVE])
#define ACT_W (!vprob || w[GCS_VI_ACTIVE])
#if defined(GCS_EMULATE)
    const int *tr = T.tile_rec + 8 * (size_t)tile;
#else
    const int *tr = (const int *)(B + L.tr);
#endif
    const int v0 = tr[0], nvt = tr[1], b0 = tr[2], nb = tr[3], h0 = tr[6], nhe = tr[7] & 0x3fffffff;
    const bool has_zero = (tr[7] >> 30) & 1;
    double *tS = B + L.tS, *eS = S + L.eS, *coneS = B + L.cone, *tnS = B + L.tnS, *enS = S + L.enS, *TS = S + L.T, *rS = S + L.r;
    double *cin = S + L.cin, *cout = S + L.cout, *vd = S + L.vd;
    int *vi = (int *)(B + L.vi), *brec = (int *)(B + L.bi);
#define bhe(b) brec[4 * (b)]
#define binfo(b) brec[4 * (b) + 1]
#define bedge(b) brec[4 * (b) + 2]
#if defined(GCS_EMULATE)
    {
        const int c0 = tr[4], ncone = tr[5];
        memcpy(tS, T.tstate + 12 * (size_t)b0, sizeof(double) * 12 * nb);
        memcpy(tnS, T.tn + 2 * (size_t)v0, sizeof(double) * 2 * nvt);
        memcpy(coneS, T.cone + GCS_CONE_REC * (size_t)c0, sizeof(double) * GCS_CONE_REC * ncone);
        memcpy(vi, T.vrec + GCS_VI_N * (size_t)v0, sizeof(int) * GCS_VI_N * nvt);
        memcpy(brec, T.blk_rec + 4 * (size_t)b0, sizeof(int) * 4 * nb);
    }
#endif
    if (vprob) {
        GCS_CTA_LOOP(i, nvt) {
            int *w = vi + GCS_VI_N * i;
            Ctrl *c = ctrl_all + w[GCS_VI_ACTIVE];
            w[GCS_VI_ACTIVE] = !(c->stop && !c->ignore_stop);
            vd[2 * i] = c->rho; vd[2 * i + 1] = c->mu_scale;
            if (w[GCS_VI_ACTIVE] && w[GCS_VI_NB]) {
#if defined(GCS_EMULATE)
                c->inner_iters += (unsigned long long)T.inner_iters;
#else
                atomicAdd(&c->inner_iters, (unsigned long long)T.inner_iters);
#endif
            }
        }
    }
#if !defined(GCS_EMULATE)
    double pz[GCS_PF], pm[GCS_PF];
#pragma unroll
    for (int j = 0; j < GCS_PF; ++j) {
        const int q = threadIdx.x + j * blockDim.x;
        pz[j] = 0.0; pm[j] = 0.0;
        if (q < 5 * nb) {
            const int b = q / 5, c = q - 5 * b, h = bhe(b);
            if (h >= 0) { pz[j] = gcs_target_z(St, T, bedge(b), c, binfo(b)); pm[j] = St.mu[5 * (size_t)h + c]; }
        }
    }
#endif
    if (vprob) GCS_CTA_SYNC();
    if (has_zero) GCS_CTA_LOOP(q, 5 * nhe) {
        const int hl = q / 5, c = q - 5 * hl, h = h0 + hl, f = G.he_flags[h];
        if (!(f & GCS_HE_ZERO)) continue;
        int vl = 0;
        while (vl + 1 < nvt && vi[GCS_VI_N * (vl + 1) + GCS_VI_HE] <= hl) ++vl;
        if (!ACT(vl)) continue;
        double x = 0.0;
        if (c < 2 && !(f & GCS_HE_OUT)) x = St.z[5 * (size_t)G.he_edge[h] + c] + MSC(vl) * St.mu[5 * (size_t)h + c];
        St.xc[5 * (size_t)h + c] = x;
    }
    const double alpha = T.alpha, kappa = T.kappa;
    for (int it = 0; it < T.inner_iters; ++it) {
        const bool last = it + 1 == T.inner_iters;
        GCS_CTA_LOOP(p, 4 * nb) {
            const int b = p >> 2, info = binfo(b), vl = info & 255;
            const int *w = vi + GCS_VI_N * vl;
            if (!ACT_W || ((info >> 10) & (p & 1))) continue;
            const double ms = it ? 1.0 : MSC(vl);
            double *t = tS + 3 * p, *e = eS + 3 * p;
            const double t0 = t[0], t1 = t[1], t2 = t[2];
            double q0, q1, q2;
            gcs_cone_project(coneS + GCS_CONE_REC * w[GCS_VI_CONE], w[GCS_VI_NV], t0, t1, t2, q0, q1, q2);
            const double l0 = ms * (t0 - q0), l1 = ms * (t1 - q1), l2 = ms * (t2 - q2);
            t[0] = q0 - l0; t[1] = q1 - l1; t[2] = q2 - l2;
            e[0] = (1.0 - alpha) * q0 + l0; e[1] = (1.0 - alpha) * q1 + l1; e[2] = (1.0 - alpha) * q2 + l2;
        }
        GCS_CTA_LOOP(i, nvt) {
            const int *w = vi + GCS_VI_N * i;
            if (!ACT_W || !w[GCS_VI_NB]) continue;
            const double ms = it ? 1.0 : MSC(i);
            const double sigma = kappa * RHO(i) * ms;
            const double a0 = tnS[2 * i], a1 = tnS[2 * i + 1], nrm = hypot(a0, a1);
            const double sc = nrm > 0.0 ? fmax(0.0, 1.0 - 1.0 / (sigma * nrm)) : 0.0;
            const double q0 = sc * a0, q1 = sc * a1, l0 = ms * (a0 - q0), l1 = ms * (a1 - q1);
            tnS[2 * i] = q0 - l0; tnS[2 * i + 1] = q1 - l1;
            enS[2 * i] = (1.0 - alpha) * q0 + l0; enS[2 * i + 1] = (1.0 - alpha) * q1 + l1;
        }
        if (it == 0) {
#if !defined(GCS_EMULATE)
#pragma unroll
            for (int j = 0; j < GCS_PF; ++j) {
                const int q = threadIdx.x + j * blockDim.x;
                if (q < 5 * nb) TS[q] = pz[j] + MSC(binfo(q / 5) & 255) * pm[j];
            }
            for (int q = threadIdx.x + GCS_PF * blockDim.x; q < 5 * nb; q += blockDim.x) {
#else
            for (int q = 0; q < 5 * nb; ++q) {
#endif
                const int b = q / 5, c = q - 5 * b, h = bhe(b), vl = binfo(b) & 255;
                if (h < 0 || !ACT(vl)) continue;
                TS[q] = gcs_target_z(St, T, bedge(b), c, binfo(b)) + MSC(vl) * St.mu[5 * (size_t)h + c];
            }
        }
        GCS_CTA_SYNC();
#if defined(GCS_EMULATE)
        for (int vl = 0; vl < nvt; ++vl) {
            const int *w = vi + GCS_VI_N * vl;
            if (!ACT_W || !w[GCS_VI_NB]) continue;
            for (int q = 5 * w[GCS_VI_BLK]; q < 5 * (w[GCS_VI_BLK] + w[GCS_VI_NB]); ++q) rS[q] = gcs_rhs(T, tS, TS, tnS, brec, q, vl, RHO(vl), kappa);
            for (int k = 0; k < GCS_NCX; ++k) cin[GCS_NCX * vl + k] = gcs_core_input(tS, rS, brec, w, k, kappa);
            for (int k = 0; k < GCS_NCX; ++k) cout[GCS_NCX * vl + k] = gcs_core_output(T.cls_tab + (size_t)GCS_CLS_STRIDE * w[GCS_VI_CLS], cin + GCS_NCX * vl, k);
        }
#else
        for (int vl = threadIdx.x >> 5; vl < nvt; vl += blockDim.x >> 5) {
            const int *w = vi + GCS_VI_N * vl;
            const int k = threadIdx.x & 31;
            if (!ACT_W || !w[GCS_VI_NB]) continue;
            for (int q = 5 * w[GCS_VI_BLK] + k; q < 5 * (w[GCS_VI_BLK] + w[GCS_VI_NB]); q += 32) rS[q] = gcs_rhs(T, tS, TS, tnS, brec, q, vl, RHO(vl), kappa);
            __syncwarp();
            if (k < GCS_NCX) cin[GCS_NCX * vl + k] = gcs_core_input(tS, rS, brec, w, k, kappa);
            __syncwarp();
            if (k < GCS_NCX) cout[GCS_NCX * vl + k] = gcs_core_output(T.cls_tab + (size_t)GCS_CLS_STRIDE * w[GCS_VI_CLS], cin + GCS_NCX * vl, k);
        }
#endif
        GCS_CTA_SYNC();
        GCS_CTA_LOOP(p, 4 * nb) {
            const int b = p >> 2, i = (p >> 1) & 1, fam = p & 1, info = binfo(b), vl = info & 255;
            const int *w = vi + GCS_VI_N * vl;
            if (!ACT_W || ((info >> 10) & fam)) continue;
            const double *co = cout + GCS_NCX * vl, *tab = T.cls_tab + (size_t)GCS_CLS_STRIDE * w[GCS_VI_CLS], *e = eS + 3 * p;
            double p0 = gcs_block_u(rS, co, tab, info, b, 2 * i), p1 = gcs_block_u(rS, co, tab, info, b, 2 * i + 1), p2 = gcs_block_u(rS, co, tab, info, b, 4);
            if (fam) { p0 = co[2 * i] - p0; p1 = co[2 * i + 1] - p1; p2 = 1.0 - p2; }
            double *t = tS + 3 * p;
            if (INNER && last) {
                const double ic = 1.0 / (2.0 - alpha), r0 = p0 - ic * (t[0] + e[0]), r1 = p1 - ic * (t[1] + e[1]), r2_ = p2 - ic * (t[2] + e[2]);
                rin += r0 * r0 + r1 * r1 + r2_ * r2_;
            }
            t[0] = alpha * p0 + e[0]; t[1] = alpha * p1 + e[1]; t[2] = alpha * p2 + e[2];
        }
        GCS_CTA_LOOP(i, nvt) {
            const int *w = vi + GCS_VI_N * i;
            if (!ACT_W || !w[GCS_VI_NB]) continue;
            const double *zz = cout + GCS_NCX * i + 4;
            if (INNER && last) {
                const double ic = 1.0 / (2.0 - alpha), r0 = (zz[0] - zz[2]) - ic * (tnS[2 * i] + enS[2 * i]), r1 = (zz[1] - zz[3]) - ic * (tnS[2 * i + 1] + enS[2 * i + 1]);
                rin += r0 * r0 + r1 * r1;
            }
            tnS[2 * i] = alpha * (zz[0] - zz[2]) + enS[2 * i]; tnS[2 * i + 1] = alpha * (zz[1] - zz[3]) + enS[2 * i + 1];
        }
        if (last) {
            GCS_CTA_LOOP(q, 9 * nvt) {
                const int vl = q / 9, k = q - 9 * vl;
                const int *w = vi + GCS_VI_N * vl;
                if (!ACT_W || !w[GCS_VI_NB]) continue;
                double val = cout[GCS_NCX * vl + k];
                const size_t v = (size_t)(v0 + vl);
                if (T.edge_delta && k < 8)
                    val += (k < 4 ? 1.0 : cout[GCS_NCX * vl + 8]) * G.cent[2 * v + (k & 1)];
                if (k < 4) St.x_v[4 * v + k] = val; else if (k < 8) St.z_v[4 * v + k - 4] = val; else St.y_v[v] = val;
            }
            GCS_CTA_LOOP(q, 5 * nb) {
                const int b = q / 5, c = q - 5 * b, h = bhe(b), info = binfo(b), vl = info & 255;
                const int *w = vi + GCS_VI_N * vl;
                if (h < 0 || !ACT_W) continue;
                const double *co = cout + GCS_NCX * vl, *tab = T.cls_tab + (size_t)GCS_CLS_STRIDE * w[GCS_VI_CLS];
                double x;
                if ((info >> 8) & 1) x = gcs_block_u(rS, co, tab, info, b, c);
                else x = c < 2 ? TS[q] : gcs_block_u(rS, co, tab, info, b, c < 4 ? c - 2 : 4);
                St.xc[5 * (size_t)h + c] = x;
            }
        }
        if (!last) GCS_CTA_SYNC();
    }
#if defined(GCS_EMULATE)
    memcpy(T.tstate + 12 * (size_t)b0, tS, sizeof(double) * 12 * nb);
    memcpy(T.tn + 2 * (size_t)v0, tnS, sizeof(double) * 2 * nvt);
    if (!vprob) ctrl_all->inner_iters += (unsigned long long)T.inner_iters * (unsigned long long)nvt;
#else
    gcs_fence_async_smem();
    GCS_CTA_SYNC();
    if (threadIdx.x == 0) {
        if (nb) gcs_bulk_s2g(T.tstate + 12 * (size_t)b0, tS, (unsigned)(sizeof(double) * 12 * nb));
        gcs_bulk_s2g(T.tn + 2 * (size_t)v0, tnS, (unsigned)(sizeof(double) * 2 * nvt));
        gcs_bulk_commit();
        if (!vprob) atomicAdd(&ctrl_all->inner_iters, (unsigned long long)T.inner_iters * (unsigned long long)nvt);
    }
#endif
#undef bhe
#undef binfo
#undef bedge
#undef RHO
#undef MSC
#undef ACT
#undef ACT_W
}
```

gcs-admm_b200/perf.py:

```python
from __future__ import annotations

import numpy as np

from .graph import _vertices_batch

NCORE, UX, UT, UZ, UYV = 10, 0, 4, 5, 9


def _uw(j):
    return NCORE + 5 * j


def _forward(v, d, jstar, prim, term, affine):
    u = np.zeros(NCORE + 5 * d)
    u[UX:UX + 4] = v[0:4]
    u[UT] = v[4]
    zy = np.zeros(5)
    other = np.zeros(5)
    if term:
        zy[0:4] = v[0:4]
        zy[4] = 1.0 if affine else 0.0
    for jj in range(d - 1):
        j = jj if jj < jstar else jj + 1
        w = v[5 + 5 * jj: 10 + 5 * jj]
        u[_uw(j):_uw(j) + 5] = w
        if prim[j]:
            other += w
        else:
            zy += w
    u[UZ:UZ + 5] = zy
    u[_uw(jstar):_uw(jstar) + 5] = zy - other
    return u


def _pair_values(u, d, term):
    npair = 4 * (d + 1)
    pv = np.zeros(3 * npair + 2)
    for blk in range(d + 1):
        for i in range(2):
            po = (_uw(blk) if blk < d else UZ) + 2 * i
            yo = _uw(blk) + 4 if blk < d else UYV
            xo = UX + 2 * i
            for fam in range(1 if term else 2):
                o = 3 * ((blk * 2 + i) * 2 + fam)
                if fam:
                    pv[o:o + 3] = (u[xo] - u[po], u[xo + 1] - u[po + 1], 1.0 - u[yo])
                else:
                    pv[o:o + 3] = (u[po], u[po + 1], u[yo])
    pv[3 * npair] = u[UZ] - u[UZ + 2]
    pv[3 * npair + 1] = u[UZ + 1] - u[UZ + 3]
    return pv


def class_pattern(vtype, din, dout):
    d = din + dout
    out = [0] * din + [1] * dout
    term = vtype != 0
    prim = [1] * d if vtype == 2 else list(out)
    jstar = max(j for j in range(d) if prim[j])
    return d, out, prim, jstar, term


def class_inverse(vtype, din, dout, kappa):
    d, out, prim, jstar, term = class_pattern(vtype, din, dout)
    n, nu = 5 * d, NCORE + 5 * d
    N = np.zeros((nu, n))
    for k in range(n):
        e = np.zeros(n); e[k] = 1.0
        N[:, k] = _forward(e, d, jstar, prim, term, False)
    pv0 = _pair_values(np.zeros(nu), d, term)
    M = np.zeros((pv0.shape[0], nu))
    for k in range(nu):
        e = np.zeros(nu); e[k] = 1.0
        M[:, k] = _pair_values(e, d, term) - pv0
    S = np.zeros(nu)
    for j in range(d):
        o = _uw(j)
        S[o:o + 2] = 1.0
        if out[j]:
            S[o + 2:o + 4] = 1.0
        S[o + 4] = 1.0
    K1 = N.T @ (np.diag(S) + kappa * M.T @ M) @ N
    K1[4, :] = 0.0; K1[:, 4] = 0.0; K1[4, 4] = 1.0
    w = np.linalg.eigvalsh(K1)
    if w[0] <= 1e-12 * w[-1]:
        raise ValueError(f"singular v-step matrix for class {(vtype, din, dout)}")
    Kinv = np.linalg.inv(K1)
    Kinv[4, :] = 0.0; Kinv[:, 4] = 0.0
    return np.ascontiguousarray(Kinv)


def cone_table(g, shift=None):
    verts, cnt = g.polygon_vertices_batch() if hasattr(g, "polygon_vertices_batch") else _vertices_batch(g.poly_off.astype(np.int64), g.polyA, g.polyb)
    if shift is not None:
        verts = verts - np.asarray(shift)[:, None, :]
    nV = g.nV
    per = [None] * nV
    for k in np.unique(cnt):
        idx = np.nonzero(cnt == k)[0]
        P = verts[idx, :k]
        c = P.mean(axis=1, keepdims=True)
        ang = np.arctan2(P[..., 1] - c[..., 1], P[..., 0] - c[..., 0])
        order = np.argsort(ang, axis=1)
        P = np.take_along_axis(P, order[..., None], axis=1)
        nxt = np.roll(P, -1, axis=1)
        dup = np.max(np.abs(P - nxt), axis=2) <= 1e-12 * np.maximum(1.0, np.abs(P).max(axis=2))
        clean = ~np.any(dup, axis=1)
        R = np.concatenate([P, np.ones(P.shape[:2] + (1,))], axis=2)
        Nn = np.cross(R, np.roll(R, -1, axis=1))
        nrm = np.linalg.norm(Nn, axis=2, keepdims=True)
        Nn = Nn / np.where(nrm > 0, nrm, 1.0)
        inner = np.concatenate([c, np.ones((c.shape[0], 1, 1))], axis=2)
        flip = np.sum(Nn * inner, axis=2) > 0
        Nn = np.where(flip[..., None], -Nn, Nn)
        Rn = np.roll(R, -1, axis=1)
        ma = np.cross(Nn, Rn); mb = np.cross(R, Nn)
        ma *= np.sign(np.sum(ma * R, axis=2, keepdims=True)); mb *= np.sign(np.sum(mb * Rn, axis=2, keepdims=True))
        rec = np.concatenate([P, Nn, 1.0 / np.sum(R * R, axis=2, keepdims=True), ma, mb], axis=2)
        for gi, v in enumerate(idx):
            per[v] = rec[gi] if clean[gi] else None
    for v in range(nV):
        if per[v] is None:
            per[v] = _cone_one(verts[v, :cnt[v]])
    off = np.zeros(nV + 1, dtype=np.int64)
    np.cumsum([p.shape[0] for p in per], out=off[1:])
    return off.astype(np.int32), np.ascontiguousarray(np.vstack(per))


def _cone_one(P):
    keep = []
    for p in P:
        if not any(np.max(np.abs(p - q)) <= 1e-12 * max(1.0, np.abs(p).max()) for q in keep):
            keep.append(p)
    P = np.array(keep)
    c = P.mean(axis=0)
    P = P[np.argsort(np.arctan2(P[:, 1] - c[1], P[:, 0] - c[0]))]
    R = np.hstack([P, np.ones((P.shape[0], 1))])
    Nn = np.cross(R, np.roll(R, -1, axis=0))
    Nn /= np.linalg.norm(Nn, axis=1, keepdims=True)
    flip = (Nn @ np.array([c[0], c[1], 1.0])) > 0
    Nn[flip] *= -1.0
    Rn = np.roll(R, -1, axis=0)
    ma = np.cross(Nn, Rn); mb = np.cross(R, Nn)
    ma *= np.sign(np.sum(ma * R, axis=1, keepdims=True)); mb *= np.sign(np.sum(mb * Rn, axis=1, keepdims=True))
    return np.hstack([P, Nn, 1.0 / np.sum(R * R, axis=1, keepdims=True), ma, mb])


CORE_IDX = (0, 1, 2, 3, 5, 6, 7, 8, 9)
NCX = 19
CLS_STRIDE = NCX * NCX + NCX + 10 + 2


def class_tables(vtype, din, dout, kappa, theta=1.0):
    d, out, prim, jstar, term = class_pattern(vtype, din, dout)
    n, nu = 5 * d, NCORE + 5 * d
    N = np.zeros((nu, n))
    for k in range(n):
        e = np.zeros(n); e[k] = 1.0
        N[:, k] = _forward(e, d, jstar, prim, term, False)
    pv0 = _pair_values(np.zeros(nu), d, term)
    M = np.zeros((pv0.shape[0], nu))
    for k in range(nu):
        e = np.zeros(nu); e[k] = 1.0
        M[:, k] = _pair_values(e, d, term) - pv0
    S = np.zeros(nu)
    for j in range(d):
        o = _uw(j)
        S[o:o + 2] = 1.0
        if out[j]:
            S[o + 2:o + 4] = 1.0
        S[o + 4] = theta
    D = np.diag(S) + kappa * M.T @ M
    K1 = N.T @ D @ N
    K1[4, :] = 0.0; K1[:, 4] = 0.0; K1[4, 4] = 1.0
    w = np.linalg.eigvalsh(K1)
    if w[0] <= 1e-12 * w[-1]:
        raise ValueError(f"singular v-step matrix for class {(vtype, din, dout)}")
    Kinv = np.linalg.inv(K1)
    Kinv[4, :] = 0.0; Kinv[:, 4] = 0.0
    Phi = N @ Kinv @ N.T
    up = _forward(np.zeros(n), d, jstar, prim, term, True)
    g0u = up - Phi @ (D @ up)
    nfam = 1 if term else 2
    dinv = np.zeros((2, 5))
    for g in range(2):
        s = np.array([1.0, 1.0, float(g), float(g), 1.0])
        dinv[g, :4] = 1.0 / (s[:4] + nfam * kappa)
        dinv[g, 4] = 1.0 / (theta + 2 * nfam * kappa)
    members = [[j for j in range(d) if not out[j]], [j for j in range(d) if out[j]]]
    G = np.zeros((NCX, NCX)); g0 = np.zeros(NCX)

    def col(k):
        if k < 9:
            return CORE_IDX[k]
        g, tau = divmod(k - 9, 5)
        return _uw(members[g][0]) + tau if members[g] else None
    for k in range(9):
        g0[k] = g0u[CORE_IDX[k]]
        for j in range(NCX):
            cj = col(j)
            if cj is not None:
                G[k, j] = Phi[CORE_IDX[k], cj]
    for g in range(2):
        if not members[g]:
            continue
        b0 = members[g][0]
        for tau in range(5):
            row = _uw(b0) + tau
            g0[9 + 5 * g + tau] = g0u[row]
            for j in range(NCX):
                if j < 9:
                    G[9 + 5 * g + tau, j] = Phi[row, CORE_IDX[j]]
                    continue
                g2, tau2 = divmod(j - 9, 5)
                if not members[g2]:
                    continue
                if g2 != g:
                    G[9 + 5 * g + tau, j] = Phi[row, _uw(members[g2][0]) + tau2]
                elif len(members[g]) >= 2:
                    G[9 + 5 * g + tau, j] = Phi[row, _uw(members[g][1]) + tau2]
                else:
                    G[9 + 5 * g + tau, j] = Phi[row, _uw(b0) + tau2] - (dinv[g, tau] if tau2 == tau else 0.0)
    return dict(G=G, g0=g0, dinv=dinv, Phi=Phi, g0u=g0u, members=members, term=term, d=d)


def structured_vstep(T, r):
    d, members = T["d"], T["members"]
    inp = np.zeros(NCX)
    inp[:9] = r[list(CORE_IDX)]
    for g in range(2):
        for j in members[g]:
            inp[9 + 5 * g:14 + 5 * g] += r[_uw(j):_uw(j) + 5]
    core = T["G"] @ inp + T["g0"]
    u = np.zeros(NCORE + 5 * d)
    u[list(CORE_IDX)] = core[:9]
    for g in range(2):
        for j in members[g]:
            u[_uw(j):_uw(j) + 5] = T["dinv"][g] * r[_uw(j):_uw(j) + 5] + core[9 + 5 * g:14 + 5 * g]
    return u


import os as _os
TILE_BLOCKS = int(_os.environ.get("GCS_TILE_BLOCKS", "64"))
TILE_THREADS = int(_os.environ.get("GCS_TILE_THREADS", str(min(256, 4 * TILE_BLOCKS))))
TILE_VERTS, TILE_CONE, TILE_HE = 32, 160, 128


def perf_tables(g, kappa=1.0, cone=None, theta=1.0, frames="global", edge_delta=None, edge_cent=None):
    nV = g.nV
    owner = np.repeat(np.arange(nV, dtype=np.int64), np.diff(np.asarray(g.he_off, dtype=np.int64)))
    flags = np.asarray(g.he_flags)
    live = (flags & 2) == 0
    outm = (flags & 1) == 1
    vtype = np.asarray(g.vtype)
    din = np.bincount(owner[live & ~outm], minlength=nV)
    dout = np.bincount(owner[live & outm], minlength=nV)
    alive = vtype != 3
    keys = {}
    vclass = np.full(nV, -1, dtype=np.int32)
    code = vtype.astype(np.int64) * 1000000 + din * 1000 + dout
    tabs = []
    for cd in np.unique(code[alive]):
        key = (int(cd // 1000000), int((cd // 1000) % 1000), int(cd % 1000))
        keys[key] = len(keys)
        T = class_tables(*key, kappa, theta)
        tabs.append(np.concatenate([np.ascontiguousarray(T["G"].T).reshape(-1), T["g0"], T["dinv"].reshape(-1), np.zeros(2)]))
        vclass[(code == cd) & alive] = keys[key]
    cls_tab = np.ascontiguousarray(np.concatenate(tabs)) if tabs else np.zeros(CLS_STRIDE)
    cent = np.asarray(g.interior_points()) if frames == "local" else None
    if cone is None:
        cone_off, cone_rec = cone_table(g, shift=cent)
    else:
        cone_off, cone_rec = cone
    if frames == "local" and edge_delta is None:
        if not hasattr(g, "edge_tail"):
            raise ValueError("local frames need edge_tail / edge_head (single-GPU graphs)")
        edge_delta = np.ascontiguousarray(cent[np.asarray(g.edge_tail, dtype=np.int64)] - cent[np.asarray(g.edge_head, dtype=np.int64)])
        edge_cent = np.ascontiguousarray(cent[np.asarray(g.edge_tail, dtype=np.int64)])
    nlive = np.where(alive, din + dout, 0).astype(np.int64)
    nblk = np.where(alive, nlive + 1, 0).astype(np.int64)
    blk_off = np.zeros(nV + 1, dtype=np.int64)
    np.cumsum(nblk, out=blk_off[1:])
    Btot = int(blk_off[-1])
    blk_he = np.full(Btot, -1, dtype=np.int32)
    blk_v = np.repeat(np.arange(nV, dtype=np.int64), nblk)
    hl = np.nonzero(live & alive[owner])[0]
    rank_in_v = np.arange(hl.shape[0]) - np.repeat(np.cumsum(nlive) - nlive, nlive)
    blk_he[blk_off[owner[hl]] + rank_in_v] = hl
    grp = np.full(Btot, 2, dtype=np.int64)
    grp[blk_off[owner[hl]] + rank_in_v] = outm[hl].astype(np.int64)
    he_cnt = np.diff(np.asarray(g.he_off, dtype=np.int64))
    cone_cnt = np.diff(np.asarray(cone_off, dtype=np.int64))
    tile_voff = _greedy_tiles(nblk, he_cnt, cone_cnt)
    tile_of_v = np.repeat(np.arange(tile_voff.shape[0] - 1), np.diff(tile_voff))
    vloc = np.arange(nV, dtype=np.int64) - tile_voff[tile_of_v]
    term = (vtype != 0)
    blk_info = (vloc[blk_v] | (grp << 8) | (term[blk_v].astype(np.int64) << 10)).astype(np.int32)
    tv0, tv1 = tile_voff[:-1], tile_voff[1:]
    caps = dict(nb=int((blk_off[tv1] - blk_off[tv0]).max()) if nV else 1, nvt=int((tv1 - tv0).max()) if nV else 1,
                cone=int((np.asarray(cone_off, np.int64)[tv1] - np.asarray(cone_off, np.int64)[tv0]).max()) if nV else 1,
                he=int((np.asarray(g.he_off, np.int64)[tv1] - np.asarray(g.he_off, np.int64)[tv0]).max()) if nV else 1)
    return dict(vclass=vclass, cls_tab=cls_tab, cone_off=np.asarray(cone_off, dtype=np.int32), cone=np.ascontiguousarray(cone_rec),
                blk_off=blk_off.astype(np.int32), blk_he=blk_he, blk_info=blk_info, tile_voff=tile_voff.astype(np.int32),
                caps=caps, classes=keys, kappa=float(kappa), theta=float(theta), edge_delta=edge_delta, edge_cent=edge_cent if frames == "local" else None,
                frames=frames, threads=TILE_THREADS)


def _greedy_tiles(nblk, he_cnt, cone_cnt):
    nV = nblk.shape[0]
    cb, ch, cc = np.concatenate([[0], np.cumsum(nblk)]), np.concatenate([[0], np.cumsum(he_cnt)]), np.concatenate([[0], np.cumsum(cone_cnt)])
    bounds = [0]
    v = 0
    while v < nV:
        e = min(int(np.searchsorted(cb, cb[v] + TILE_BLOCKS, side="right")) - 1,
                int(np.searchsorted(ch, ch[v] + TILE_HE, side="right")) - 1,
                int(np.searchsorted(cc, cc[v] + TILE_CONE, side="right")) - 1, v + TILE_VERTS, nV)
        e = max(e, v + 1)
        bounds.append(e)
        v = e
    return np.array(bounds, dtype=np.int64)


def local_tables(T, lp):
    lv = np.asarray(lp.global_vertices, dtype=np.int64)
    off = T["cone_off"].astype(np.int64)
    cnt = off[lv + 1] - off[lv]
    loff = np.zeros(lv.shape[0] + 1, dtype=np.int64)
    np.cumsum(cnt, out=loff[1:])
    rec = T["cone"].reshape(-1, 12)
    idx = np.repeat(off[lv] - loff[:-1], cnt) + np.arange(int(loff[-1]))
    frames = T.get("frames", "global")
    delta = np.ascontiguousarray(T["edge_delta"][np.asarray(lp.global_edges, dtype=np.int64)]) if frames == "local" else None
    ecent = np.ascontiguousarray(T["edge_cent"][np.asarray(lp.global_edges, dtype=np.int64)]) if frames == "local" and T.get("edge_cent") is not None else None
    return perf_tables(lp, T["kappa"], cone=(loff.astype(np.int32), np.ascontiguousarray(rec[idx])), theta=T.get("theta", 1.0), frames=frames, edge_delta=delta,
                       edge_cent=ecent)
```

Measured before the change: 3558.

## Split perf tile into cone and gather warp groups, batch cone projections, specialize batch mode

The perf tile kernel now splits each CTA into two warp groups. One group projects both cone points of a block together, sharing each cone-ray load between them. The other group runs the norm prox and the first-iteration target gathers at the same time. Prefetch of the next tile moves inside the tile loop onto a dedicated copy thread. Batch mode becomes a template parameter, which removes runtime vprob branches. The inner-iteration counter is now updated once per launch instead of one atomic per tile. Vertex records also carry the in-block count, so core_input avoids scanning block groups; this relies on blocks being ordered in, out, then z, which is now validated on the host.

After: 4040 (median of 6 runs). 13.6% higher.

```diff
diff --git a/gcs-admm_b200/csrc/emulate.cpp b/gcs-admm_b200/csrc/emulate.cpp
--- a/gcs-admm_b200/csrc/emulate.cpp
+++ b/gcs-admm_b200/csrc/emulate.cpp
@@ -53,7 +53,9 @@
         for (int v = a; v < b; ++v) {
             int *w = vrec + GCS_VI_N * v;
             w[GCS_VI_CONE] = cone_off[v] - cone_off[a]; w[GCS_VI_NV] = cone_off[v + 1] - cone_off[v]; w[GCS_VI_CLS] = vclass[v];
-            w[GCS_VI_TERM] = vtype[v] != GCS_VT_GENERIC; w[GCS_VI_BLK] = blk_off[v] - blk_off[a]; w[GCS_VI_NB] = blk_off[v + 1] - blk_off[v];
+            int nin = 0;
+            for (int bb = blk_off[v]; bb < blk_off[v + 1]; ++bb) nin += ((blk_info[bb] >> 8) & 3) == 0;
+            w[GCS_VI_TERM] = (vtype[v] != GCS_VT_GENERIC) | (nin << 1); w[GCS_VI_BLK] = blk_off[v] - blk_off[a]; w[GCS_VI_NB] = blk_off[v + 1] - blk_off[v];
             w[GCS_VI_ACTIVE] = 0; w[GCS_VI_HE] = he_off[v] - he_off[a];
         }
     }
@@ -70,7 +72,7 @@
             memset(S, poison, sizeof(double) * L.total);
             Ctrl local = ctrl;
             double rin = 0.0;
-            gcs_perf_tile<INNER>(G, St, T, L, S, S + L.work, t, &local, 0, rin);
+            gcs_perf_tile<INNER, false>(G, St, T, L, S, S + L.work, t, &local, rin, nullptr, 0, nullptr);
             if (rin_tile) rin_tile[t] = rin;
         }
         free(S);
@@ -116,3 +118,10 @@
 extern "C" void gcsemu_cone_project(const double *cone, int nv, const double *pts, int n, double *out) {
     for (int i = 0; i < n; ++i) gcs_cone_project(cone, nv, pts[3 * i], pts[3 * i + 1], pts[3 * i + 2], out[3 * i], out[3 * i + 1], out[3 * i + 2]);
 }
+extern "C" void gcsemu_cone_project2(const double *cone, int nv, const double *pts, int n, double *out) {
+    for (int i = 0; i + 1 < n; i += 2) {
+        const double *c = pts + 3 * i;
+        double *q = out + 3 * i;
+        gcs_cone_project2(cone, nv, c[0], c[1], c[2], c[3], c[4], c[5], q[0], q[1], q[2], q[3], q[4], q[5]);
+    }
+}
diff --git a/gcs-admm_b200/csrc/gcsadmm.cu b/gcs-admm_b200/csrc/gcsadmm.cu
--- a/gcs-admm_b200/csrc/gcsadmm.cu
+++ b/gcs-admm_b200/csrc/gcsadmm.cu
@@ -133,12 +133,15 @@
     __syncthreads();
 }
 
-template <bool INNER>
+template <bool INNER, bool BATCH>
 __global__ void __launch_bounds__(GCS_PERF_THREADS, 4)
-vertex_perf_kernel(GcsGraphView G, GcsStateView St, GcsPerfTables T, Ctrl *ctrl_all, const int *__restrict__ vprob, GcsPerfLayout L, PeerPush P) {
+vertex_perf_kernel(GcsGraphView G, GcsStateView St, GcsPerfTables T, Ctrl *ctrl_all, GcsPerfLayout L, PeerPush P) {
     extern __shared__ __align__(16) double smem[];
     __shared__ __align__(8) unsigned long long bar[2];
-    if (!vprob && ctrl_all->stop && !ctrl_all->ignore_stop) return;
+    if (!BATCH) {
+        if (ctrl_all->stop && !ctrl_all->ignore_stop) return;
+        if (blockIdx.x == 0 && threadIdx.x == 0) atomicAdd(&ctrl_all->inner_iters, (unsigned long long)T.inner_iters * (unsigned long long)G.nV);
+    }
     int tile = blockIdx.x;
     if (tile >= T.ntiles) return;
     double *const stage0 = smem + L.work;
@@ -149,19 +152,13 @@
         gcs_perf_stage(T, L, STAGE(0), tile, &bar[0]);
     }
     __syncthreads();
-    unsigned phase = 0;
     double rin = 0.0;
-    for (int buf = 0; tile < T.ntiles; tile += gridDim.x, buf ^= 1) {
-        const int next = tile + gridDim.x;
-        if (threadIdx.x == 0 && next < T.ntiles) {
-            gcs_bulk_wait_read();
-            gcs_perf_stage(T, L, STAGE(buf ^ 1), next, &bar[buf ^ 1]);
-        }
-        gcs_mbar_wait(&bar[buf], (phase >> buf) & 1u);
-        phase ^= 1u << buf;
-        gcs_perf_tile<INNER>(G, St, T, L, smem, STAGE(buf), tile, ctrl_all, vprob, rin);
-    }
-    if (threadIdx.x == 0) gcs_bulk_wait_read();
+    for (unsigned n = 0; tile < T.ntiles; tile += gridDim.x, ++n) {
+        const int buf = n & 1;
+        gcs_mbar_wait(&bar[buf], (n >> 1) & 1u);
+        gcs_perf_tile<INNER, BATCH>(G, St, T, L, smem, STAGE(buf), tile, ctrl_all, rin, STAGE(buf ^ 1), tile + gridDim.x, &bar[buf ^ 1]);
+    }
+    if (threadIdx.x == GCS_COPY_THREAD) gcs_bulk_wait_read();
 #undef STAGE
     if (INNER) {
 #pragma unroll
@@ -820,8 +817,9 @@
 static int launch_k1(GcsHandle *h) {
     if (h->perf_on) {
         PeerPush P = {h->send_he, h->send_rank, h->send_slot, h->nsend, h->peer_on ? h->PV_dev : nullptr, h->push_ticket};
-        if (h->inner_on) vertex_perf_kernel<true><<<h->perf_grid, h->perf_threads, h->perf_smem, h->stream>>>(graph_view(h), state_view(h), h->PT, h->ctrl, h->vprob, h->PL, P);
-        else vertex_perf_kernel<false><<<h->perf_grid, h->perf_threads, h->perf_smem, h->stream>>>(graph_view(h), state_view(h), h->PT, h->ctrl, h->vprob, h->PL, P);
+        auto *k = h->vprob ? (h->inner_on ? vertex_perf_kernel<true, true> : vertex_perf_kernel<false, true>)
+                           : (h->inner_on ? vertex_perf_kernel<true, false> : vertex_perf_kernel<false, false>);
+        k<<<h->perf_grid, h->perf_threads, h->perf_smem, h->stream>>>(graph_view(h), state_view(h), h->PT, h->ctrl, h->PL, P);
         return 0;
     }
     vertex_kernel<<<h->k1_blocks, h->k1_warps * 32, h->k1_smem, h->stream>>>(graph_view(h), state_view(h), h->ctrl, h->vprob, h->L, h->p.inner_tol, h->p.inner_max_iter);
@@ -1259,7 +1257,7 @@
             for (size_t b = 0; b < nB; ++b) {
                 brec[4 * b] = c->blk_he[b]; brec[4 * b + 1] = c->blk_info[b]; brec[4 * b + 2] = c->blk_he[b] >= 0 ? he_edge[c->blk_he[b]] : -1;
             }
-            for (int t = 0; t < c->n_tiles; ++t) {
+            for (int t = 0; t < c->n_tiles && !rc; ++t) {
                 const int a = c->tile_voff[t], b = c->tile_voff[t + 1];
                 int *r = trec + 8 * (size_t)t;
                 r[0] = a; r[1] = b - a; r[2] = c->blk_off[a]; r[3] = c->blk_off[b] - c->blk_off[a];
@@ -1267,15 +1265,21 @@
                 bool zero = false;
                 for (int hh = he_off[a]; hh < he_off[b]; ++hh) zero = zero || (he_flags[hh] & GCS_HE_FLAG_ZERO);
                 if (zero) r[7] |= 1 << 30;
-                for (int v = a; v < b; ++v) {
+                for (int v = a; v < b && !rc; ++v) {
+                    int nin = 0, g = 0;
+                    for (int bb = c->blk_off[v]; bb < c->blk_off[v + 1]; ++bb) {
+                        const int gb = (c->blk_info[bb] >> 8) & 3;
+                        if (gb < g || (gb == 2) != (bb == c->blk_off[v + 1] - 1)) rc = set_err(GCS_E_INVALID, "perf-mode blocks of a vertex are not in-, out-, z-block order%s", "");
+                        g = gb; nin += gb == 0;
+                    }
                     int *w = vrec + GCS_VI_N * (size_t)v;
                     w[GCS_VI_CONE] = c->cone_off[v] - c->cone_off[a]; w[GCS_VI_NV] = c->cone_off[v + 1] - c->cone_off[v];
-                    w[GCS_VI_CLS] = c->vclass[v]; w[GCS_VI_TERM] = vtype[v] != GCS_VT_GENERIC;
+                    w[GCS_VI_CLS] = c->vclass[v]; w[GCS_VI_TERM] = (vtype[v] != GCS_VT_GENERIC) | (nin << 1);
                     w[GCS_VI_BLK] = c->blk_off[v] - c->blk_off[a]; w[GCS_VI_NB] = c->blk_off[v + 1] - c->blk_off[v];
                     w[GCS_VI_ACTIVE] = vprob[v]; w[GCS_VI_HE] = he_off[v] - he_off[a];
                 }
             }
-            rc = upload(&h->p_blk_rec, brec, 4 * nB);
+            if (!rc) rc = upload(&h->p_blk_rec, brec, 4 * nB);
             if (!rc) rc = upload(&h->p_vrec, vrec, GCS_VI_N * nVt);
             if (!rc) rc = upload(&h->p_tile_rec, trec, 8 * nT);
         }
@@ -1307,10 +1311,10 @@
         const long long cap = (long long)prop.multiProcessorCount * per_sm;
         h->perf_grid = (int)(c->n_tiles < cap ? c->n_tiles : cap);
     }
-    CK(cudaFuncSetAttribute(vertex_perf_kernel<false>, cudaFuncAttributeMaxDynamicSharedMemorySize, h->perf_smem));
-    CK(cudaFuncSetAttribute(vertex_perf_kernel<false>, cudaFuncAttributePreferredSharedMemoryCarveout, 100));
-    CK(cudaFuncSetAttribute(vertex_perf_kernel<true>, cudaFuncAttributeMaxDynamicSharedMemorySize, h->perf_smem));
-    CK(cudaFuncSetAttribute(vertex_perf_kernel<true>, cudaFuncAttributePreferredSharedMemoryCarveout, 100));
+    for (auto *k : {vertex_perf_kernel<false, false>, vertex_perf_kernel<true, false>, vertex_perf_kernel<false, true>, vertex_perf_kernel<true, true>}) {
+        CK(cudaFuncSetAttribute(k, cudaFuncAttributeMaxDynamicSharedMemorySize, h->perf_smem));
+        CK(cudaFuncSetAttribute(k, cudaFuncAttributePreferredSharedMemoryCarveout, 100));
+    }
     perf_init_dead_kernel<<<(h->nV + 255) / 256, 256, 0, h->stream>>>(graph_view(h), state_view(h));
     CK(cudaGetLastError());
     CK(cudaStreamSynchronize(h->stream));
diff --git a/gcs-admm_b200/csrc/vertex_perf.cuh b/gcs-admm_b200/csrc/vertex_perf.cuh
--- a/gcs-admm_b200/csrc/vertex_perf.cuh
+++ b/gcs-admm_b200/csrc/vertex_perf.cuh
@@ -78,30 +78,34 @@
     return L;
 }
 
-GCS_DEV void gcs_cone_project(const double *cone, int nv, double c0, double c1, double c2, double &q0, double &q1, double &q2) {
-    double best = 0.0;
-    int code = -1;
-    bool inside = true;
-    for (int k = 0; k < nv; ++k) {
-#if defined(GCS_EMULATE)
-        const double *r = cone + GCS_CONE_REC * k;
-        const double vx = r[0], vy = r[1], nx = r[2], ny = r[3], nh = r[4], inv = r[5], a0 = r[6], a1 = r[7], a2 = r[8], b0 = r[9], b1 = r[10], b2 = r[11];
-#else
-        const double2 *r = reinterpret_cast<const double2 *>(cone + GCS_CONE_REC * k);
-        const double2 r0 = r[0], r1 = r[1], r2 = r[2], r3 = r[3], r4 = r[4], r5 = r[5];
-        const double vx = r0.x, vy = r0.y, nx = r1.x, ny = r1.y, nh = r2.x, inv = r2.y, a0 = r3.x, a1 = r3.y, a2 = r4.x, b0 = r4.y, b1 = r5.x, b2 = r5.y;
-#endif
-        const double tau = c0 * vx + c1 * vy + c2;
-        const double dist = nx * c0 + ny * c1 + nh * c2;
-        if (tau > 0.0) {
-            const double red = tau * tau * inv;
-            if (red > best) { best = red; code = 2 * k; }
-        }
-        if (dist > 0.0) {
-            inside = false;
-            if (c0 * a0 + c1 * a1 + c2 * a2 >= 0.0 && c0 * b0 + c1 * b1 + c2 * b2 >= 0.0) { best = 1e300; code = 2 * k + 1; }
-        }
-    }
+struct GcsConeRay { double vx, vy, nx, ny, nh, inv; };
+#if defined(GCS_EMULATE)
+GCS_DEV GcsConeRay gcs_cone_ray(const double *cone, int k) { const double *r = cone + GCS_CONE_REC * k; return GcsConeRay{r[0], r[1], r[2], r[3], r[4], r[5]}; }
+#else
+GCS_DEV GcsConeRay gcs_cone_ray(const double *cone, int k) {
+    const double2 *r = reinterpret_cast<const double2 *>(cone + GCS_CONE_REC * k);
+    const double2 r0 = r[0], r1 = r[1], r2 = r[2];
+    return GcsConeRay{r0.x, r0.y, r1.x, r1.y, r2.x, r2.y};
+}
+#endif
+GCS_DEV double gcs_cone_sector_dot(const double *cone, int k, int s, double c0, double c1, double c2) {
+    const double *m = cone + GCS_CONE_REC * k + 6 + 3 * s;
+    return c0 * m[0] + c1 * m[1] + c2 * m[2];
+}
+GCS_DEV double gcs_cone_test_ray(const GcsConeRay &R, int k, double c0, double c1, double c2, double &best, int &code) {
+    const double tau = c0 * R.vx + c1 * R.vy + c2;
+    const double dist = R.nx * c0 + R.ny * c1 + R.nh * c2;
+    if (tau > 0.0) {
+        const double red = tau * tau * R.inv;
+        if (red > best) { best = red; code = 2 * k; }
+    }
+    return dist;
+}
+GCS_DEV void gcs_cone_take_face(bool sector, int k, double &best, int &code, bool &inside) {
+    inside = false;
+    if (sector) { best = 1e300; code = 2 * k + 1; }
+}
+GCS_DEV void gcs_cone_pick(const double *cone, int code, bool inside, double c0, double c1, double c2, double &q0, double &q1, double &q2) {
     if (inside) { q0 = c0; q1 = c1; q2 = c2; return; }
     q0 = 0.0; q1 = 0.0; q2 = 0.0;
     if (code < 0) return;
@@ -114,6 +118,37 @@
         q0 = tau * ck[0]; q1 = tau * ck[1]; q2 = tau;
     }
 }
+GCS_DEV void gcs_cone_project(const double *cone, int nv, double c0, double c1, double c2, double &q0, double &q1, double &q2) {
+    double best = 0.0;
+    int code = -1;
+    bool inside = true;
+#pragma unroll 1
+    for (int k = 0; k < nv; ++k) {
+        const double dist = gcs_cone_test_ray(gcs_cone_ray(cone, k), k, c0, c1, c2, best, code);
+        if (dist > 0.0) gcs_cone_take_face(gcs_cone_sector_dot(cone, k, 0, c0, c1, c2) >= 0.0 && gcs_cone_sector_dot(cone, k, 1, c0, c1, c2) >= 0.0, k, best, code, inside);
+    }
+    gcs_cone_pick(cone, code, inside, c0, c1, c2, q0, q1, q2);
+}
+GCS_DEV void gcs_cone_project2(const double *cone, int nv, double c0, double c1, double c2, double d0, double d1, double d2,
+                               double &q0, double &q1, double &q2, double &s0, double &s1, double &s2) {
+    double best_c = 0.0, best_d = 0.0;
+    int code_c = -1, code_d = -1;
+    bool inside_c = true, inside_d = true;
+#pragma unroll 1
+    for (int k = 0; k < nv; ++k) {
+        const GcsConeRay R = gcs_cone_ray(cone, k);
+        const double dist_c = gcs_cone_test_ray(R, k, c0, c1, c2, best_c, code_c);
+        const double dist_d = gcs_cone_test_ray(R, k, d0, d1, d2, best_d, code_d);
+        if (dist_c > 0.0 || dist_d > 0.0) {
+            const bool ma_c = gcs_cone_sector_dot(cone, k, 0, c0, c1, c2) >= 0.0, ma_d = gcs_cone_sector_dot(cone, k, 0, d0, d1, d2) >= 0.0;
+            const bool mb_c = gcs_cone_sector_dot(cone, k, 1, c0, c1, c2) >= 0.0, mb_d = gcs_cone_sector_dot(cone, k, 1, d0, d1, d2) >= 0.0;
+            if (dist_c > 0.0) gcs_cone_take_face(ma_c && mb_c, k, best_c, code_c, inside_c);
+            if (dist_d > 0.0) gcs_cone_take_face(ma_d && mb_d, k, best_d, code_d, inside_d);
+        }
+    }
+    gcs_cone_pick(cone, code_c, inside_c, c0, c1, c2, q0, q1, q2);
+    gcs_cone_pick(cone, code_d, inside_d, d0, d1, d2, s0, s1, s2);
+}
 
 #if !defined(GCS_EMULATE) && defined(__CUDACC__)
 __device__ __forceinline__ unsigned gcs_smem_u32(const void *p) { return (unsigned)__cvta_generic_to_shared(p); }
@@ -145,15 +180,15 @@
 
 #define GCS_PF 3
 
-GCS_DEV double gcs_core_input(const double *tS, const double *rS, const int *brec, const int *w, int k, double kappa) {
+GCS_DEV double gcs_core_input(const double *tS, const double *rS, const int *w, int k, double kappa) {
     const int bl = w[GCS_VI_BLK], zb = bl + w[GCS_VI_NB] - 1;
     double s = 0.0;
     if (k < 4) {
-        if (!w[GCS_VI_TERM]) { for (int b = bl; b <= zb; ++b) s += tS[12 * b + 6 * (k >> 1) + 3 + (k & 1)]; s *= kappa; }
+        if (!(w[GCS_VI_TERM] & 1)) { for (int b = bl; b <= zb; ++b) s += tS[12 * b + 6 * (k >> 1) + 3 + (k & 1)]; s *= kappa; }
     } else if (k < 9) s = rS[5 * zb + k - 4];
     else {
-        const int g = k >= 14, tau = k - 9 - 5 * g;
-        for (int b = bl; b < zb; ++b) if (((brec[4 * b + 1] >> 8) & 3) == g) s += rS[5 * b + tau];
+        const int g = k >= 14, tau = k - 9 - 5 * g, bin = bl + (w[GCS_VI_TERM] >> 1);
+        for (int b = g ? bin : bl; b < (g ? zb : bin); ++b) s += rS[5 * b + tau];
     }
     return s;
 }
@@ -198,7 +233,9 @@
     return zc;
 }
 
+
 #if !defined(GCS_EMULATE) && defined(__CUDACC__)
+#define GCS_COPY_THREAD (blockDim.x - 32)
 __device__ __forceinline__ void gcs_perf_stage(const GcsPerfTables &T, const GcsPerfLayout &L, double *B, int tile, unsigned long long *bar) {
     const int *tr = T.tile_rec + 8 * (size_t)tile;
     const int v0 = tr[0], nvt = tr[1], b0 = tr[2], nb = tr[3], c0 = tr[4], ncone = tr[5];
@@ -212,14 +249,21 @@
 }
 #endif
 
-template <bool INNER>
+GCS_DEV void gcs_cstep_store(double *t, double *e, double t0, double t1, double t2, double q0, double q1, double q2, double ms, double alpha) {
+    const double l0 = ms * (t0 - q0), l1 = ms * (t1 - q1), l2 = ms * (t2 - q2);
+    t[0] = q0 - l0; t[1] = q1 - l1; t[2] = q2 - l2;
+    e[0] = (1.0 - alpha) * q0 + l0; e[1] = (1.0 - alpha) * q1 + l1; e[2] = (1.0 - alpha) * q2 + l2;
+}
+
+template <bool INNER, bool BATCH>
 GCS_DEV void gcs_perf_tile(const GcsGraphView &G, const GcsStateView &St, const GcsPerfTables &T, const GcsPerfLayout &L,
-                           double *S, double *B, int tile, Ctrl *ctrl_all, const int *vprob, double &rin) {
+                           double *S, double *B, int tile, Ctrl *ctrl_all, double &rin,
+                           double *Bn, int next, unsigned long long *bar_next) {
     const double rho_u = ctrl_all->rho, ms_u = ctrl_all->mu_scale;
-#define RHO(vl) (vprob ? vd[2 * (vl)] : rho_u)
-#define MSC(vl) (vprob ? vd[2 * (vl) + 1] : ms_u)
-#define ACT(vl) (!vprob || vi[GCS_VI_N * (vl) + GCS_VI_ACTIVE])
-#define ACT_W (!vprob || w[GCS_VI_ACTIVE])
+#define RHO(vl) (BATCH ? vd[2 * (vl)] : rho_u)
+#define MSC(vl) (BATCH ? vd[2 * (vl) + 1] : ms_u)
+#define ACT(vl) (!BATCH || vi[GCS_VI_N * (vl) + GCS_VI_ACTIVE])
+#define ACT_W (!BATCH || w[GCS_VI_ACTIVE])
 #if defined(GCS_EMULATE)
     const int *tr = T.tile_rec + 8 * (size_t)tile;
 #else
@@ -243,7 +287,15 @@
         memcpy(brec, T.blk_rec + 4 * (size_t)b0, sizeof(int) * 4 * nb);
     }
 #endif
-    if (vprob) {
+#if defined(GCS_EMULATE)
+    const bool cgrp = true, ggrp = true;
+    const int cid = 0, cn = 1, gid0 = 0, gn = 1;
+#else
+    const int nw = blockDim.x >> 5, cn = 32 * ((nw + 1) >> 1);
+    const bool cgrp = (int)threadIdx.x < cn, ggrp = !cgrp || nw == 1;
+    const int cid = threadIdx.x, gid0 = nw == 1 ? (int)threadIdx.x : (int)threadIdx.x - cn, gn = nw == 1 ? cn : (int)blockDim.x - cn;
+#endif
+    if (BATCH) {
         GCS_CTA_LOOP(i, nvt) {
             int *w = vi + GCS_VI_N * i;
             Ctrl *c = ctrl_all + w[GCS_VI_ACTIVE];
@@ -257,80 +309,101 @@
 #endif
             }
         }
-    }
-#if !defined(GCS_EMULATE)
-    double pz[GCS_PF], pm[GCS_PF];
-#pragma unroll
-    for (int j = 0; j < GCS_PF; ++j) {
-        const int q = threadIdx.x + j * blockDim.x;
-        pz[j] = 0.0; pm[j] = 0.0;
-        if (q < 5 * nb) {
-            const int b = q / 5, c = q - 5 * b, h = bhe(b);
-            if (h >= 0) { pz[j] = gcs_target_z(St, T, bedge(b), c, binfo(b)); pm[j] = St.mu[5 * (size_t)h + c]; }
-        }
-    }
-#endif
-    if (vprob) GCS_CTA_SYNC();
-    if (has_zero) GCS_CTA_LOOP(q, 5 * nhe) {
-        const int hl = q / 5, c = q - 5 * hl, h = h0 + hl, f = G.he_flags[h];
-        if (!(f & GCS_HE_ZERO)) continue;
-        int vl = 0;
-        while (vl + 1 < nvt && vi[GCS_VI_N * (vl + 1) + GCS_VI_HE] <= hl) ++vl;
-        if (!ACT(vl)) continue;
-        double x = 0.0;
-        if (c < 2 && !(f & GCS_HE_OUT)) x = St.z[5 * (size_t)G.he_edge[h] + c] + MSC(vl) * St.mu[5 * (size_t)h + c];
-        St.xc[5 * (size_t)h + c] = x;
+        GCS_CTA_SYNC();
     }
     const double alpha = T.alpha, kappa = T.kappa;
     for (int it = 0; it < T.inner_iters; ++it) {
         const bool last = it + 1 == T.inner_iters;
-        GCS_CTA_LOOP(p, 4 * nb) {
-            const int b = p >> 2, info = binfo(b), vl = info & 255;
+        if (ggrp) {
+#if defined(GCS_EMULATE)
+            const int gid = gid0;
+#else
+            int gid = gid0;
+            asm volatile("" : "+r"(gid));
+#endif
+            if (it == 0 && has_zero) for (int q = gid; q < 5 * nhe; q += gn) {
+                const int hl = q / 5, c = q - 5 * hl, h = h0 + hl, f = G.he_flags[h];
+                if (!(f & GCS_HE_ZERO)) continue;
+                int vl = 0;
+                while (vl + 1 < nvt && vi[GCS_VI_N * (vl + 1) + GCS_VI_HE] <= hl) ++vl;
+                if (!ACT(vl)) continue;
+                double x = 0.0;
+                if (c < 2 && !(f & GCS_HE_OUT)) x = St.z[5 * (size_t)G.he_edge[h] + c] + MSC(vl) * St.mu[5 * (size_t)h + c];
+                St.xc[5 * (size_t)h + c] = x;
+            }
+            for (int i = gid; i < nvt; i += gn) {
+                const int *w = vi + GCS_VI_N * i;
+                if (!ACT_W || !w[GCS_VI_NB]) continue;
+                const double ms = it ? 1.0 : MSC(i);
+                const double sigma = kappa * RHO(i) * ms;
+                const double a0 = tnS[2 * i], a1 = tnS[2 * i + 1], nrm = hypot(a0, a1);
+                const double sc = nrm > 0.0 ? fmax(0.0, 1.0 - 1.0 / (sigma * nrm)) : 0.0;
+                const double q0 = sc * a0, q1 = sc * a1, l0 = ms * (a0 - q0), l1 = ms * (a1 - q1);
+                tnS[2 * i] = q0 - l0; tnS[2 * i + 1] = q1 - l1;
+                enS[2 * i] = (1.0 - alpha) * q0 + l0; enS[2 * i + 1] = (1.0 - alpha) * q1 + l1;
+            }
+#if !defined(GCS_EMULATE)
+            double pz[GCS_PF], pm[GCS_PF];
+            if (it == 0) {
+#pragma unroll
+                for (int j = 0; j < GCS_PF; ++j) {
+                    const int q = gid + j * gn;
+                    pz[j] = 0.0; pm[j] = 0.0;
+                    if (q < 5 * nb) {
+                        const int b = q / 5, c = q - 5 * b, h = bhe(b);
+                        if (h >= 0) { pz[j] = gcs_target_z(St, T, bedge(b), c, binfo(b)); pm[j] = St.mu[5 * (size_t)h + c]; }
+                    }
+                }
+            }
+#endif
+            if (it == 0) {
+#if !defined(GCS_EMULATE)
+#pragma unroll
+                for (int j = 0; j < GCS_PF; ++j) {
+                    const int q = gid + j * gn;
+                    if (q < 5 * nb) TS[q] = pz[j] + MSC(binfo(q / 5) & 255) * pm[j];
+                }
+                for (int q = gid + GCS_PF * gn; q < 5 * nb; q += gn) {
+#else
+                for (int q = 0; q < 5 * nb; ++q) {
+#endif
+                    const int b = q / 5, c = q - 5 * b, h = bhe(b), vl = binfo(b) & 255;
+                    if (h < 0 || !ACT(vl)) continue;
+                    TS[q] = gcs_target_z(St, T, bedge(b), c, binfo(b)) + MSC(vl) * St.mu[5 * (size_t)h + c];
+                }
+            }
+        }
+        if (cgrp) for (int j = cid; j < 2 * nb; j += cn) {
+            const int b = j >> 1, info = binfo(b), vl = info & 255;
             const int *w = vi + GCS_VI_N * vl;
-            if (!ACT_W || ((info >> 10) & (p & 1))) continue;
+            if (!ACT_W) continue;
             const double ms = it ? 1.0 : MSC(vl);
-            double *t = tS + 3 * p, *e = eS + 3 * p;
+            const double *cone = coneS + GCS_CONE_REC * w[GCS_VI_CONE];
+            double *t = tS + 6 * j, *e = eS + 6 * j;
             const double t0 = t[0], t1 = t[1], t2 = t[2];
             double q0, q1, q2;
-            gcs_cone_project(coneS + GCS_CONE_REC * w[GCS_VI_CONE], w[GCS_VI_NV], t0, t1, t2, q0, q1, q2);
-            const double l0 = ms * (t0 - q0), l1 = ms * (t1 - q1), l2 = ms * (t2 - q2);
-            t[0] = q0 - l0; t[1] = q1 - l1; t[2] = q2 - l2;
-            e[0] = (1.0 - alpha) * q0 + l0; e[1] = (1.0 - alpha) * q1 + l1; e[2] = (1.0 - alpha) * q2 + l2;
-        }
-        GCS_CTA_LOOP(i, nvt) {
-            const int *w = vi + GCS_VI_N * i;
-            if (!ACT_W || !w[GCS_VI_NB]) continue;
-            const double ms = it ? 1.0 : MSC(i);
-            const double sigma = kappa * RHO(i) * ms;
-            const double a0 = tnS[2 * i], a1 = tnS[2 * i + 1], nrm = hypot(a0, a1);
-            const double sc = nrm > 0.0 ? fmax(0.0, 1.0 - 1.0 / (sigma * nrm)) : 0.0;
-            const double q0 = sc * a0, q1 = sc * a1, l0 = ms * (a0 - q0), l1 = ms * (a1 - q1);
-            tnS[2 * i] = q0 - l0; tnS[2 * i + 1] = q1 - l1;
-            enS[2 * i] = (1.0 - alpha) * q0 + l0; enS[2 * i + 1] = (1.0 - alpha) * q1 + l1;
-        }
-        if (it == 0) {
+            if ((info >> 10) & 1) gcs_cone_project(cone, w[GCS_VI_NV], t0, t1, t2, q0, q1, q2);
+            else {
+                const double t3 = t[3], t4 = t[4], t5 = t[5];
+                double q3, q4, q5;
+                gcs_cone_project2(cone, w[GCS_VI_NV], t0, t1, t2, t3, t4, t5, q0, q1, q2, q3, q4, q5);
+                gcs_cstep_store(t + 3, e + 3, t3, t4, t5, q3, q4, q5, ms, alpha);
+            }
+            gcs_cstep_store(t, e, t0, t1, t2, q0, q1, q2, ms, alpha);
+        }
+        GCS_CTA_SYNC();
 #if !defined(GCS_EMULATE)
-#pragma unroll
-            for (int j = 0; j < GCS_PF; ++j) {
-                const int q = threadIdx.x + j * blockDim.x;
-                if (q < 5 * nb) TS[q] = pz[j] + MSC(binfo(q / 5) & 255) * pm[j];
-            }
-            for (int q = threadIdx.x + GCS_PF * blockDim.x; q < 5 * nb; q += blockDim.x) {
-#else
-            for (int q = 0; q < 5 * nb; ++q) {
-#endif
-                const int b = q / 5, c = q - 5 * b, h = bhe(b), vl = binfo(b) & 255;
-                if (h < 0 || !ACT(vl)) continue;
-                TS[q] = gcs_target_z(St, T, bedge(b), c, binfo(b)) + MSC(vl) * St.mu[5 * (size_t)h + c];
-            }
-        }
-        GCS_CTA_SYNC();
+        if (it == 0 && threadIdx.x == GCS_COPY_THREAD && next < T.ntiles) {
+            gcs_bulk_wait_read();
+            gcs_perf_stage(T, L, Bn, next, bar_next);
+        }
+#endif
 #if defined(GCS_EMULATE)
         for (int vl = 0; vl < nvt; ++vl) {
             const int *w = vi + GCS_VI_N * vl;
             if (!ACT_W || !w[GCS_VI_NB]) continue;
             for (int q = 5 * w[GCS_VI_BLK]; q < 5 * (w[GCS_VI_BLK] + w[GCS_VI_NB]); ++q) rS[q] = gcs_rhs(T, tS, TS, tnS, brec, q, vl, RHO(vl), kappa);
-            for (int k = 0; k < GCS_NCX; ++k) cin[GCS_NCX * vl + k] = gcs_core_input(tS, rS, brec, w, k, kappa);
+            for (int k = 0; k < GCS_NCX; ++k) cin[GCS_NCX * vl + k] = gcs_core_input(tS, rS, w, k, kappa);
             for (int k = 0; k < GCS_NCX; ++k) cout[GCS_NCX * vl + k] = gcs_core_output(T.cls_tab + (size_t)GCS_CLS_STRIDE * w[GCS_VI_CLS], cin + GCS_NCX * vl, k);
         }
 #else
@@ -340,7 +413,7 @@
             if (!ACT_W || !w[GCS_VI_NB]) continue;
             for (int q = 5 * w[GCS_VI_BLK] + k; q < 5 * (w[GCS_VI_BLK] + w[GCS_VI_NB]); q += 32) rS[q] = gcs_rhs(T, tS, TS, tnS, brec, q, vl, RHO(vl), kappa);
             __syncwarp();
-            if (k < GCS_NCX) cin[GCS_NCX * vl + k] = gcs_core_input(tS, rS, brec, w, k, kappa);
+            if (k < GCS_NCX) cin[GCS_NCX * vl + k] = gcs_core_input(tS, rS, w, k, kappa);
             __syncwarp();
             if (k < GCS_NCX) cout[GCS_NCX * vl + k] = gcs_core_output(T.cls_tab + (size_t)GCS_CLS_STRIDE * w[GCS_VI_CLS], cin + GCS_NCX * vl, k);
         }
@@ -397,15 +470,13 @@
 #if defined(GCS_EMULATE)
     memcpy(T.tstate + 12 * (size_t)b0, tS, sizeof(double) * 12 * nb);
     memcpy(T.tn + 2 * (size_t)v0, tnS, sizeof(double) * 2 * nvt);
-    if (!vprob) ctrl_all->inner_iters += (unsigned long long)T.inner_iters * (unsigned long long)nvt;
 #else
     gcs_fence_async_smem();
     GCS_CTA_SYNC();
-    if (threadIdx.x == 0) {
+    if (threadIdx.x == GCS_COPY_THREAD) {
         if (nb) gcs_bulk_s2g(T.tstate + 12 * (size_t)b0, tS, (unsigned)(sizeof(double) * 12 * nb));
         gcs_bulk_s2g(T.tn + 2 * (size_t)v0, tnS, (unsigned)(sizeof(double) * 2 * nvt));
         gcs_bulk_commit();
-        if (!vprob) atomicAdd(&ctrl_all->inner_iters, (unsigned long long)T.inner_iters * (unsigned long long)nvt);
     }
 #endif
 #undef bhe
diff --git a/gcs-admm_b200/perf.py b/gcs-admm_b200/perf.py
--- a/gcs-admm_b200/perf.py
+++ b/gcs-admm_b200/perf.py
@@ -289,6 +289,8 @@
     blk_he[blk_off[owner[hl]] + rank_in_v] = hl
     grp = np.full(Btot, 2, dtype=np.int64)
     grp[blk_off[owner[hl]] + rank_in_v] = outm[hl].astype(np.int64)
+    if Btot and not np.all((np.diff(grp) >= 0) | (np.diff(blk_v) != 0)):
+        raise ValueError("perf tables need every vertex's in-half-edges before its out-half-edges")
     he_cnt = np.diff(np.asarray(g.he_off, dtype=np.int64))
     cone_cnt = np.diff(np.asarray(cone_off, dtype=np.int64))
     tile_voff = _greedy_tiles(nblk, he_cnt, cone_cnt)
```
